# mozilla/mozjpeg

Hardware: AMD Instinct MI355X
Metric: Mpixels/s encode (4K RGB q75 trellis) at 1/2/4/8 GPUs; bit-exact vs cjpeg (higher is better)
Workload: dtype u8/int16 (+f32 trellis costs); 1 GPU; 3840x2160 synthetic RGB, q75 4:2:0 baseline, trellis+deringing+optimal Huffman (cjpeg -quality 75 -baseline); config_key=metric, frames_per_encode_call=96, distinct_frames=96, batches_in_flight=2, input=resident in HBM, output=complete JPEG files in HBM, parallelism=images sharded, 1 process per GPU, no collective

## Files before the change

### include/mozjpeg_hip.h

```cpp
#ifndef MOZJPEG_HIP_H
#define MOZJPEG_HIP_H

#include <stddef.h>
#include <stdint.h>

#ifdef __cplusplus
extern "C" {
#endif

#define MJH_MAX_COMPS 4
#define MJH_MAX_SCANS 64

#define MJH_OK            0
#define MJH_EINVAL       -1
#define MJH_EUNSUPPORTED -2
#define MJH_EHIP         -3
#define MJH_ENOMEM       -4
#define MJH_ETOOSMALL    -5

#define MJH_PROFILE_MAX_COMPRESSION 0x5D083AAD
#define MJH_PROFILE_FASTEST         0x2AEA5CB4

typedef struct {
  int comps_in_scan;
// ... 51 lines not shown

int mjh_std_huffman_table(int is_ac, int tblno, const uint8_t **bits, const uint8_t **vals, int *nvals);

int mjh_params_simple_progression(mjh_params *p);
int mjh_params_search_progression(mjh_params *p);

int mjh_encoder_create(const mjh_params *p, int max_batch, int device, mjh_encoder **out);
int mjh_device_count(void);
int mjh_device_numa_node(int device);
int mjh_bind_thread_to_device(int device);
int mjh_device_placement(int device, char *buf, size_t n);
void mjh_encoder_destroy(mjh_encoder *e);
const mjh_params *mjh_encoder_params(const mjh_encoder *e);

typedef struct mjh_pool mjh_pool;
int mjh_pool_create(const mjh_params *p, int max_batch_per_device, const int *devices, int ndevices, mjh_pool **out);
void mjh_pool_destroy(mjh_pool *pool);
int mjh_pool_device_count(const mjh_pool *pool);
int mjh_pool_encode_host(mjh_pool *pool, const void *pixels, size_t row_pitch, size_t image_stride, int n,
                         const uint8_t *const **jpegs, const size_t **sizes);
const char *mjh_pool_last_error(const mjh_pool *pool);

int mjh_encode_device(mjh_encoder *e, const void *d_pixels, size_t row_pitch, size_t image_stride,
                      int n, void *stream);
int mjh_set_inflight(mjh_encoder *e, int batches);
int mjh_encode_host(mjh_encoder *e, const void *pixels, size_t row_pitch, size_t image_stride, int n);
typedef struct { uint64_t offset, size; } mjh_result;
int mjh_collect(mjh_encoder *e, int age, const void **base, const mjh_result **results, int *count);
int mjh_wait_input(mjh_encoder *e);
int mjh_host_staging(mjh_encoder *e, void **buffer, size_t *bytes);
int mjh_stage_commit(mjh_encoder *e, size_t bytes);
int mjh_encode_gather(mjh_encoder *e, mjh_encoder *const *members, int n);
void *mjh_host_alloc(size_t bytes);
void mjh_host_free(void *p);
int mjh_host_register(void *p, size_t bytes);
int mjh_host_unregister(void *p);
int mjh_encode_planes_device(mjh_encoder *e, const void *const d_planes[MJH_MAX_COMPS], const size_t row_pitch[MJH_MAX_COMPS],
                             const size_t image_stride[MJH_MAX_COMPS], const int plane_width[MJH_MAX_COMPS],
                             const int plane_height[MJH_MAX_COMPS], int n, void *stream);
int mjh_encode_planes_host(mjh_encoder *e, const void *const planes[MJH_MAX_COMPS], const size_t row_pitch[MJH_MAX_COMPS],
                           const size_t image_stride[MJH_MAX_COMPS], const int plane_width[MJH_MAX_COMPS],
                           const int plane_height[MJH_MAX_COMPS], int n);
int mjh_encode_coefficients_device(mjh_encoder *e, const void *const d_coefs[MJH_MAX_COMPS], const size_t blocks_per_row[MJH_MAX_COMPS],
                                   const size_t image_stride[MJH_MAX_COMPS], int n, void *stream);
int mjh_encode_coefficients_host(mjh_encoder *e, const void *const coefs[MJH_MAX_COMPS], const size_t blocks_per_row[MJH_MAX_COMPS],
                                 const size_t image_stride[MJH_MAX_COMPS], int n);
int mjh_encoder_sync(mjh_encoder *e);

#define MJH_MAX_FILE_SCANS 4
#define MJH_CS_GRAYSCALE 1
#define MJH_CS_RGB       2
#define MJH_CS_YCbCr     3
typedef struct {
  int comps_in_scan;
  int component_index[MJH_MAX_COMPS];
  int dc_tbl_no[MJH_MAX_COMPS], ac_tbl_no[MJH_MAX_COMPS];
  unsigned restart_interval;
  size_t data_offset, data_size;
  unsigned restart_markers;
  int huff_defined;
  uint8_t huff_bits[8][17];
  uint8_t huff_vals[8][256];
} mjh_jpeg_scan;
typedef struct {
  int sof_type;
  int data_precision;
  int image_width, image_height;
  int num_components;
  int component_id[MJH_MAX_COMPS], h_samp_factor[MJH_MAX_COMPS], v_samp_factor[MJH_MAX_COMPS], quant_tbl_no[MJH_MAX_COMPS];
  int quant_defined;
  uint16_t quantval[4][64];
  int jpeg_color_space;
  int saw_JFIF_marker, JFIF_major_version, JFIF_minor_version, density_unit, X_density, Y_density;
  int saw_Adobe_marker, Adobe_transform;
  int num_scans;
  mjh_jpeg_scan scans[MJH_MAX_FILE_SCANS];
} mjh_jpeg_info;
int mjh_jpeg_probe(const void *jpeg, size_t size, mjh_jpeg_info *info);
int mjh_params_from_jpeg(const mjh_jpeg_info *info, int compress_profile, mjh_params *p);
int mjh_transcode_host(mjh_encoder *e, const void *const jpegs[], const size_t sizes[], int n);
int mjh_transcode_status(mjh_encoder *e, int i, const char **text);
int mjh_transcode_stats(mjh_encoder *e, int *subseq, int *rounds, int *host_syncs, float ms[4]);

int mjh_get_jpeg_size(mjh_encoder *e, int i, size_t *size);
int mjh_get_jpeg(mjh_encoder *e, int i, void *dst, size_t cap, size_t *size);
int mjh_get_output_device(mjh_encoder *e, void **d_base, size_t *stride, void **d_sizes);

int mjh_get_scan_table(mjh_encoder *e, int image, int scan, int tblno, uint8_t bits[17], uint8_t vals[256]);

enum {
  MJH_TAP_PLANE = 1,
  MJH_TAP_COEF_UQ = 2,
  MJH_TAP_COEF_Q = 3,
  MJH_TAP_COEF_Q0 = 4,
  MJH_TAP_HUFF_BITS = 5,
  MJH_TAP_HUFF_VALS = 6,
  MJH_TAP_PROG_SCAN_US = 7,
  MJH_TAP_LL_COUNTS = 8
};
int mjh_set_debug_taps(mjh_encoder *e, int on);
int mjh_read_tap(mjh_encoder *e, int what, int image, int component, void *dst, size_t cap, size_t *size);
int mjh_component_geometry(const mjh_encoder *e, int c, int *width_in_blocks, int *height_in_blocks,
                           int *plane_width, int *plane_height);

int mjh_set_profiling(mjh_encoder *e, int level);
int mjh_set_profiling_focus(mjh_encoder *e, const char *name);
int mjh_get_kernel_times(mjh_encoder *e, const char *const **names, const float **ms, int *count);

int mjh_debug_guard_mode(void);
int mjh_debug_guard_check(void);
int mjh_debug_guard_selftest(long offset, int write);

const char *mjh_last_error(void);
const char *mjh_version(void);
size_t mjh_params_size(void);

#ifdef __cplusplus
}
#endif
#endif
```

### mozjpeg_amd/__init__.py

```python
import ctypes as C
import os

import numpy as np

_HERE = os.path.dirname(os.path.abspath(__file__))
LIB_PATH = os.environ.get("MOZJPEG_AMD_LIB") or os.path.join(_HERE, "libmozjpeg_hip.so")

MAX_COMPS, MAX_SCANS = 4, 64
PROFILE_MAX_COMPRESSION = 0x5D083AAD
PROFILE_FASTEST = 0x2AEA5CB4
COLOR_YCC, COLOR_NONE, COLOR_YCC_IN = 0, 1, 2
CS_GRAYSCALE, CS_RGB, CS_YCBCR = 1, 2, 3
OK, EINVAL, EUNSUPPORTED, EHIP, ENOMEM, ETOOSMALL = 0, -1, -2, -3, -4, -5
TAP_PLANE, TAP_COEF_UQ, TAP_COEF_Q, TAP_COEF_Q0, TAP_HUFF_BITS, TAP_HUFF_VALS, TAP_PROG_SCAN_US, TAP_LL_COUNTS = 1, 2, 3, 4, 5, 6, 7, 8


class MjhError(RuntimeError):
    def __init__(self, code, msg):
        super().__init__("mozjpeg_hip error %d: %s" % (code, msg))
        self.code = code


class Scan(C.Structure):
    _fields_ = [("comps_in_scan", C.c_int), ("component_index", C.c_int * MAX_COMPS),
# ... 31 lines not shown
class JpegInfo(C.Structure):
    _fields_ = [("sof_type", C.c_int), ("data_precision", C.c_int), ("image_width", C.c_int), ("image_height", C.c_int),
                ("num_components", C.c_int), ("component_id", C.c_int * MAX_COMPS), ("h_samp_factor", C.c_int * MAX_COMPS),
                ("v_samp_factor", C.c_int * MAX_COMPS), ("quant_tbl_no", C.c_int * MAX_COMPS), ("quant_defined", C.c_int),
                ("quantval", (C.c_uint16 * 64) * 4), ("jpeg_color_space", C.c_int), ("saw_JFIF_marker", C.c_int),
                ("JFIF_major_version", C.c_int), ("JFIF_minor_version", C.c_int), ("density_unit", C.c_int),
                ("X_density", C.c_int), ("Y_density", C.c_int), ("saw_Adobe_marker", C.c_int), ("Adobe_transform", C.c_int),
                ("num_scans", C.c_int), ("scans", JpegScan * 4)]


class Result(C.Structure):
    _fields_ = [("offset", C.c_uint64), ("size", C.c_uint64)]


_lib = None


def lib():
    global _lib
    if _lib is None:
        if not os.path.exists(LIB_PATH):
            raise MjhError(EHIP, "%s not built: run `python -m mozjpeg_amd.build` (needs hipcc)" % LIB_PATH)
        L = C.CDLL(LIB_PATH)
        L.mjh_last_error.restype = C.c_char_p
        L.mjh_version.restype = C.c_char_p
        L.mjh_params_size.restype = C.c_size_t
        if L.mjh_params_size() != C.sizeof(Params):
            raise MjhError(EINVAL, "%s (%s) has a %d-byte mjh_params, this binding a %d-byte one: rebuild"
                           % (LIB_PATH, L.mjh_version().decode(), L.mjh_params_size(), C.sizeof(Params)))
        L.mjh_device_placement.argtypes = [C.c_int, C.c_char_p, C.c_size_t]
        L.mjh_params_defaults.argtypes = [C.POINTER(Params)] + [C.c_int] * 7
        L.mjh_params_set_quality.argtypes = [C.POINTER(Params), C.c_int, C.c_int, C.c_int]
        L.mjh_params_simple_progression.argtypes = [C.POINTER(Params)]
        L.mjh_params_search_progression.argtypes = [C.POINTER(Params)]
        L.mjh_encoder_create.argtypes = [C.POINTER(Params), C.c_int, C.c_int, C.POINTER(C.c_void_p)]
        L.mjh_encoder_destroy.argtypes = [C.c_void_p]
        L.mjh_encoder_destroy.restype = None
        L.mjh_encode_device.argtypes = [C.c_void_p, C.c_void_p, C.c_size_t, C.c_size_t, C.c_int, C.c_void_p]
        L.mjh_encode_host.argtypes = [C.c_void_p, C.c_void_p, C.c_size_t, C.c_size_t, C.c_int]
        L.mjh_encode_planes_device.argtypes = [C.c_void_p] + [C.c_void_p] * 5 + [C.c_int, C.c_void_p]
        L.mjh_encode_planes_host.argtypes = [C.c_void_p] + [C.c_void_p] * 5 + [C.c_int]
        L.mjh_encode_coefficients_device.argtypes = [C.c_void_p] + [C.c_void_p] * 3 + [C.c_int, C.c_void_p]
        L.mjh_encode_coefficients_host.argtypes = [C.c_void_p] + [C.c_void_p] * 3 + [C.c_int]
        L.mjh_encoder_sync.argtypes = [C.c_void_p]
        L.mjh_set_inflight.argtypes = [C.c_void_p, C.c_int]
        L.mjh_encoder_params.argtypes = [C.c_void_p]
        L.mjh_encoder_params.restype = C.POINTER(Params)
        L.mjh_pool_create.argtypes = [C.POINTER(Params), C.c_int, C.POINTER(C.c_int), C.c_int, C.POINTER(C.c_void_p)]
        L.mjh_pool_destroy.argtypes = [C.c_void_p]
        L.mjh_pool_destroy.restype = None
        L.mjh_pool_device_count.argtypes = [C.c_void_p]
        L.mjh_pool_encode_host.argtypes = [C.c_void_p, C.c_void_p, C.c_size_t, C.c_size_t, C.c_int,
                                           C.POINTER(C.POINTER(C.c_void_p)), C.POINTER(C.POINTER(C.c_size_t))]
        L.mjh_pool_last_error.argtypes = [C.c_void_p]
        L.mjh_pool_last_error.restype = C.c_char_p
        L.mjh_collect.argtypes = [C.c_void_p, C.c_int, C.POINTER(C.c_void_p), C.POINTER(C.POINTER(Result)), C.POINTER(C.c_int)]
        L.mjh_wait_input.argtypes = [C.c_void_p]
        L.mjh_host_staging.argtypes = [C.c_void_p, C.POINTER(C.c_void_p), C.POINTER(C.c_size_t)]
        L.mjh_stage_commit.argtypes = [C.c_void_p, C.c_size_t]
        L.mjh_encode_gather.argtypes = [C.c_void_p, C.POINTER(C.c_void_p), C.c_int]
        L.mjh_host_alloc.argtypes = [C.c_size_t]
        L.mjh_host_alloc.restype = C.c_void_p
        L.mjh_host_free.argtypes = [C.c_void_p]
        L.mjh_host_free.restype = None
        L.mjh_host_register.argtypes = [C.c_void_p, C.c_size_t]
        L.mjh_host_unregister.argtypes = [C.c_void_p]
        L.mjh_get_jpeg_size.argtypes = [C.c_void_p, C.c_int, C.POINTER(C.c_size_t)]
        L.mjh_get_jpeg.argtypes = [C.c_void_p, C.c_int, C.c_void_p, C.c_size_t, C.POINTER(C.c_size_t)]
        L.mjh_get_output_device.argtypes = [C.c_void_p, C.POINTER(C.c_void_p), C.POINTER(C.c_size_t),
                                            C.POINTER(C.c_void_p)]
        L.mjh_set_debug_taps.argtypes = [C.c_void_p, C.c_int]
        L.mjh_set_profiling.argtypes = [C.c_void_p, C.c_int]
        L.mjh_set_profiling_focus.argtypes = [C.c_void_p, C.c_char_p]
        L.mjh_read_tap.argtypes = [C.c_void_p, C.c_int, C.c_int, C.c_int, C.c_void_p, C.c_size_t,
                                   C.POINTER(C.c_size_t)]
        L.mjh_component_geometry.argtypes = [C.c_void_p, C.c_int] + [C.POINTER(C.c_int)] * 4
        L.mjh_get_kernel_times.argtypes = [C.c_void_p, C.POINTER(C.POINTER(C.c_char_p)),
                                           C.POINTER(C.POINTER(C.c_float)), C.POINTER(C.c_int)]
        L.mjh_jpeg_probe.argtypes = [C.c_char_p, C.c_size_t, C.POINTER(JpegInfo)]
        L.mjh_params_from_jpeg.argtypes = [C.POINTER(JpegInfo), C.c_int, C.POINTER(Params)]
        L.mjh_transcode_host.argtypes = [C.c_void_p, C.POINTER(C.c_char_p), C.POINTER(C.c_size_t), C.c_int]
        L.mjh_transcode_status.argtypes = [C.c_void_p, C.c_int, C.POINTER(C.c_char_p)]
        L.mjh_transcode_stats.argtypes = [C.c_void_p, C.POINTER(C.c_int), C.POINTER(C.c_int), C.POINTER(C.c_int), C.POINTER(C.c_float)]
        _lib = L
    return _lib


def _chk(rc):
    if rc != 0:
        raise MjhError(rc, lib().mjh_last_error().decode())


def make_params(width, height, *, quality=75, baseline=False, revert=False, optimize=False,
                notrellis=False, notrellis_dc=False, noovershoot=False, sample=(2, 2), gray=False,
                grayin=False, quant_table=-1, lambda1=None, lambda2=None, restart=None,
                progressive=False, fastcrush=False, precision=8, trellis_loops=1, smooth=0, rgb=False,
                dc_scan_opt=None, dc_ver_weight=None, use_scans_in_trellis=False, trellis_freq_split=0,
                trellis_eob_opt=False, trellis_q_opt=False, arithmetic=False, arith_cond=None, scans=None, gray_sample=None, yccin=False, dct=None,
                dc_tbl=None, ac_tbl=None, no_optimize=False, lossless=None):
    p = Params()
    L = lib()
    per_comp = isinstance(sample[0], (tuple, list))
    s0 = sample[0] if per_comp else sample
    _chk(L.mjh_params_defaults(C.byref(p), width, height, 1 if grayin else 3, 1 if gray else 0,
                               PROFILE_FASTEST if revert else PROFILE_MAX_COMPRESSION, s0[0], s0[1]))
    if per_comp and p.num_components == 3:
        for i in range(3):
            p.h_samp_factor[i], p.v_samp_factor[i] = sample[i]
    if gray_sample is not None and p.num_components == 1:
        p.h_samp_factor[0], p.v_samp_factor[0] = gray_sample
    _chk(L.mjh_params_set_quality(C.byref(p), quality, 1 if baseline else 0, quant_table))
    for i in range(p.num_components):
        if dc_tbl is not None:
            p.dc_tbl_no[i] = dc_tbl[i]
        if ac_tbl is not None:
            p.ac_tbl_no[i] = ac_tbl[i]
        for is_ac, t in ((0, p.dc_tbl_no[i]), (1, p.ac_tbl_no[i])):
            if t > 1 and (dc_tbl is not None or ac_tbl is not None):
                bits, vals, nv = C.POINTER(C.c_uint8)(), C.POINTER(C.c_uint8)(), C.c_int()
                _chk(L.mjh_std_huffman_table(is_ac, t & 1, C.byref(bits), C.byref(vals), C.byref(nv)))
                k = 2 * t + is_ac
                for j in range(17):
                    p.huff_bits[k][j] = bits[j]
                for j in range(nv.value):
                    p.huff_vals[k][j] = vals[j]
                p.huff_tables_given |= 1 << k
    if optimize:
        p.optimize_coding = 1
    if no_optimize:
        p.optimize_coding = 0
    if notrellis:
        p.trellis_quant = 0
    if notrellis_dc:
        p.trellis_quant_dc = 0
    if noovershoot:
        p.overshoot_deringing = 0
    if lambda1 is not None:
        p.lambda_log_scale1 = lambda1
    if lambda2 is not None:
        p.lambda_log_scale2 = lambda2
    p.data_precision = precision
    p.trellis_num_loops = trellis_loops
    p.smoothing_factor = smooth
    if dc_scan_opt is not None:
        p.dc_scan_opt_mode = dc_scan_opt
    if dc_ver_weight is not None:
        p.trellis_delta_dc_weight = dc_ver_weight
    p.use_scans_in_trellis = 1 if use_scans_in_trellis else 0
    p.trellis_freq_split = trellis_freq_split
    p.trellis_eob_opt = 1 if trellis_eob_opt else 0
    p.trellis_q_opt = 1 if trellis_q_opt else 0
    p.arith_code = 1 if arithmetic else 0
    if dct == "fast":
        p.dct_method = 1
    if arith_cond is not None:
        for t, (lo, up, kx) in enumerate(arith_cond):
            p.arith_dc_L[t], p.arith_dc_U[t], p.arith_ac_K[t] = lo, up, kx
    if yccin and not grayin:
        p.color_transform = COLOR_YCC_IN
    if rgb:
        p.color_transform = COLOR_NONE
        p.write_JFIF_header = 0
        for i, cid in enumerate(b"RGB"):
            p.component_id[i] = cid
            p.h_samp_factor[i] = p.v_samp_factor[i] = 1
            p.quant_tbl_no[i] = p.dc_tbl_no[i] = p.ac_tbl_no[i] = 0
# ... 212 lines not shown
        out = []
        for i in range(cnt.value):
            mv = (C.c_uint8 * res[i].size).from_address(base.value + res[i].offset)
            out.append(bytes(mv) if copy else memoryview(mv))
        return out

    def encode_device_ptr(self, ptr, row_pitch, image_stride, n, stream=None):
        _chk(lib().mjh_encode_device(self._h, ptr, row_pitch, image_stride, n, stream))

    def encode_tensor(self, t, stream=None):
        import torch
        p = self.params
        px = p.input_pixel_size or p.input_components
        es = 2 if p.data_precision > 8 else 1
        assert t.is_cuda and t.dim() == 4 and t.element_size() == es and t.stride(3) == 1 and t.stride(2) == t.shape[3], "layout"
        assert tuple(t.shape[1:]) == (p.image_height, p.image_width, px), "tensor %s does not match the encoder (%d x %d x %d)" % (
            tuple(t.shape), p.image_height, p.image_width, px)
        assert 1 <= t.shape[0] <= self.max_batch
        if stream is None:
            stream = torch.cuda.current_stream(t.device).cuda_stream or 1
        elif stream == "own":
            stream = None
        self.encode_device_ptr(t.data_ptr(), t.stride(1) * es, t.stride(0) * es, t.shape[0], stream)

    @staticmethod
    def _plane_args(ptrs, pitches, strides, widths, heights):
        k = len(ptrs)
        pad = lambda v, z: list(v) + [z] * (4 - k)
        return ((C.c_void_p * 4)(*pad(ptrs, None)), (C.c_size_t * 4)(*pad(pitches, 0)), (C.c_size_t * 4)(*pad(strides, 0)),
                (C.c_int * 4)(*pad(widths, 0)), (C.c_int * 4)(*pad(heights, 0)))

    def encode_planes_host(self, planes):
        dt = np.uint16 if self.params.data_precision == 12 else np.uint8
        arrs = [np.ascontiguousarray(a if a.ndim == 3 else a[None], dtype=dt) for a in planes]
        n = arrs[0].shape[0]
        args = self._plane_args([a.ctypes.data for a in arrs], [a.strides[1] for a in arrs], [a.strides[0] for a in arrs],
                                [a.shape[2] for a in arrs], [a.shape[1] for a in arrs])
        _chk(lib().mjh_encode_planes_host(self._h, *args, n))
        return [self.get_jpeg(i) for i in range(n)]

    def encode_planes_tensors(self, planes, stream=None):
        for t in planes:
            assert t.is_cuda and t.dim() == 3 and t.stride(2) == 1
        es = planes[0].element_size()
        n = planes[0].shape[0]
        args = self._plane_args([t.data_ptr() for t in planes], [t.stride(1) * es for t in planes],
                                [t.stride(0) * es for t in planes], [t.shape[2] for t in planes], [t.shape[1] for t in planes])
        _chk(lib().mjh_encode_planes_device(self._h, *args, n, stream))

    def encode_coefficients_host(self, coefs):
        arrs = [np.ascontiguousarray(a if a.ndim == 4 else a[None], dtype=np.int16) for a in coefs]
        n, k = arrs[0].shape[0], len(arrs)
        pad = lambda v, z: list(v) + [z] * (4 - k)
        _chk(lib().mjh_encode_coefficients_host(self._h, (C.c_void_p * 4)(*pad([a.ctypes.data for a in arrs], None)),
                                                (C.c_size_t * 4)(*pad([a.shape[2] for a in arrs], 0)),
                                                (C.c_size_t * 4)(*pad([a.strides[0] for a in arrs], 0)), n))
        return [self.get_jpeg(i) for i in range(n)]

    def encode_coefficients_tensors(self, coefs, stream=None):
        for t in coefs:
            assert t.is_cuda and t.is_contiguous() and t.dim() == 4 and t.element_size() == 2
        n, k = coefs[0].shape[0], len(coefs)
        pad = lambda v, z: list(v) + [z] * (4 - k)
        _chk(lib().mjh_encode_coefficients_device(self._h, (C.c_void_p * 4)(*pad([t.data_ptr() for t in coefs], None)),
                                                  (C.c_size_t * 4)(*pad([t.shape[2] for t in coefs], 0)),
                                                  (C.c_size_t * 4)(*pad([t.stride(0) * 2 for t in coefs], 0)), n, stream))

    def submit_transcode(self, files):
        files = [bytes(f) for f in files]
        n = len(files)
        _chk(lib().mjh_transcode_host(self._h, (C.c_char_p * n)(*files), (C.c_size_t * n)(*[len(f) for f in files]), n))
        return n

    def transcode_status(self, i):
        t = C.c_char_p()
        rc = lib().mjh_transcode_status(self._h, i, C.byref(t))
        return rc, (t.value or b"").decode()

    def transcode_stats(self):
        a, b, c, ms = C.c_int(), C.c_int(), C.c_int(), (C.c_float * 4)()
        _chk(lib().mjh_transcode_stats(self._h, C.byref(a), C.byref(b), C.byref(c), ms))
        return dict(subseq=a.value, rounds=b.value, host_syncs=c.value, ms=dict(zip(("sync", "prefix", "store", "dc"), [float(x) for x in ms])))

    def transcode_host(self, files, errors="raise"):
        n = len(files)
        try:
            self.submit_transcode(files)
            return [self.get_jpeg(i) for i in range(n)]
        except MjhError:
            if errors != "return":
                raise
            res = []
            for i in range(n):
                rc, text = self.transcode_status(i)
                res.append(MjhError(rc, text) if rc != OK else None)
            if all(r is None for r in res):
                raise
            return res

    def set_inflight(self, batches):
        _chk(lib().mjh_set_inflight(self._h, batches))

    def sync(self):
        _chk(lib().mjh_encoder_sync(self._h))

    def get_jpeg(self, i):
        n = C.c_size_t()
        _chk(lib().mjh_get_jpeg_size(self._h, i, C.byref(n)))
        buf = np.empty(n.value, np.uint8)
        _chk(lib().mjh_get_jpeg(self._h, i, buf.ctypes.data, n.value, C.byref(n)))
        return buf.tobytes()

    def jpeg_size(self, i):
        n = C.c_size_t()
        _chk(lib().mjh_get_jpeg_size(self._h, i, C.byref(n)))
        return n.value

    def set_debug_taps(self, on=True):
        _chk(lib().mjh_set_debug_taps(self._h, int(on)))

    def set_profiling(self, on=True, focus=None):
        if focus is not None:
            _chk(lib().mjh_set_profiling_focus(self._h, focus.encode()))
        _chk(lib().mjh_set_profiling(self._h, int(on)))

    def geometry(self, c):
        v = [C.c_int() for _ in range(4)]
        _chk(lib().mjh_component_geometry(self._h, c, *[C.byref(x) for x in v]))
        return tuple(x.value for x in v)

    def read_tap(self, what, image=0, comp=0):
        wib, hib, pw, ph = self.geometry(comp if what not in (TAP_HUFF_BITS, TAP_HUFF_VALS, TAP_PROG_SCAN_US) else 0)
        if what == TAP_PROG_SCAN_US:
            out = np.zeros((2, 72), np.uint32)
        elif what == TAP_PLANE:
            out = np.empty((ph, pw), np.uint8)
        elif what == TAP_HUFF_BITS:
            out = np.empty((4, 17), np.uint8)
        elif what == TAP_HUFF_VALS:
            out = np.empty((4, 256), np.uint8)
        else:
            out = np.empty((64, wib * hib), np.int16)
        n = C.c_size_t()
        _chk(lib().mjh_read_tap(self._h, what, image, comp, out.ctypes.data, out.nbytes, C.byref(n)))
        return out

    def kernel_times(self):
        names = C.POINTER(C.c_char_p)()
        ms = C.POINTER(C.c_float)()
        cnt = C.c_int()
        _chk(lib().mjh_get_kernel_times(self._h, C.byref(names), C.byref(ms), C.byref(cnt)))
        return [(names[i].decode(), float(ms[i])) for i in range(cnt.value)]
```

### mozjpeg_amd/csrc/mjh_device.h

```cpp
#ifndef MJH_DEVICE_H
#define MJH_DEVICE_H
#ifndef MJH_SIMT_HOST
#define MJH_DIVERGENT_SCOPE
#define MJH_WAVE_GROUPS(n) ((void)0)
#define MJH_WAVE_SYNC() ((void)0)
#define MJH_SCHED_BARRIER() __builtin_amdgcn_sched_barrier(0)
#endif
#include <hip/hip_runtime.h>
#include <stdint.h>
#include "mjh_internal.h"

__device__ __forceinline__ int bitlen(unsigned v) { return 32 - __clz((int)v); }

__device__ __forceinline__ int mul24(int a, int b) { return __mul24(a, b); }
__device__ __forceinline__ float squaref(int v) { const float f = (float)v; return f * f; }

__device__ __forceinline__ int udiv_exact(int n, int d, float rcp)
{
  int q = (int)((float)n * rcp);
  int r = n - mul24(q, d);
  if (r < 0) q--; else if (r >= d) q++;
  return q;
}

// ... 70 lines not shown
  return (unsigned)x;
}

__device__ __forceinline__ unsigned block_excl_scan_256_1b(unsigned v, unsigned *sh, int parity, unsigned *total)
{
  const int lane = threadIdx.x & 63, w = threadIdx.x >> 6;
  const unsigned inc = wave_incl_scan(v);
  if (lane == 63) sh[parity * 4 + w] = inc;
  __syncthreads();
  const unsigned a = sh[parity * 4], b = sh[parity * 4 + 1], c = sh[parity * 4 + 2], d = sh[parity * 4 + 3];
  *total = a + b + c + d;
  return (w == 0 ? 0u : (w == 1 ? a : (w == 2 ? a + b : a + b + c))) + inc - v;
}


struct BitWriter {
  unsigned *words;
  unsigned long long acc;
  int nacc;
  unsigned widx;
  __device__ __forceinline__ void init(unsigned *w, unsigned bitoff) { words = w; widx = bitoff >> 5; nacc = (int)(bitoff & 31); acc = 0; }
  __device__ __forceinline__ void put(unsigned code, int n)
  {
    acc = (acc << n) | (unsigned long long)(code & ((1u << n) - 1u));
    nacc += n;
    if (nacc >= 32) {
      const unsigned w = (unsigned)(acc >> (nacc - 32));
      atomicOr(&words[widx], __builtin_bswap32(w));
      widx++;
      nacc -= 32;
    }
  }
  __device__ __forceinline__ void put_sym(unsigned e, unsigned val, int nbits)
  {
    const int n = (int)(e >> 16) + nbits;
    acc = (acc << n) | (unsigned long long)(((e & 0xFFFFu) << nbits) | (val & ((1u << nbits) - 1u)));
    nacc += n;
    if (nacc >= 32) {
      const unsigned w = (unsigned)(acc >> (nacc - 32));
      atomicOr(&words[widx], __builtin_bswap32(w));
      widx++;
      nacc -= 32;
    }
  }
  __device__ __forceinline__ void flush()
  {
    if (nacc > 0) {
      const unsigned w = (unsigned)(acc << (32 - nacc));
      atomicOr(&words[widx], __builtin_bswap32(w));
    }
  }
};


#define STUFF_LDS_WORDS (4096 + 2)
__device__ __forceinline__ void stuff_store_round(uint8_t *__restrict__ o, unsigned dst0, unsigned total, unsigned my_dst, const unsigned (&w)[8],
                                                  int nvalid, unsigned keep, unsigned *lds)
{
  uint8_t *l8 = reinterpret_cast<uint8_t *>(lds);
  const unsigned shift = (unsigned)((uintptr_t)(o + dst0) & 3u);
  unsigned at = my_dst - dst0 + shift;
#pragma unroll
  for (int i = 0; i < 8; i++) {
#pragma unroll
    for (int b = 0; b < 4; b++) {
      const unsigned byte = (w[i] >> (8 * b)) & 0xFFu;
      if (4 * i + b < nvalid) {
        l8[at++] = (uint8_t)byte;
        if (byte == 0xFFu && !((keep >> (4 * i + b)) & 1u)) l8[at++] = 0;
      }
    }
  }
  __syncthreads();
  uint8_t *g = o + dst0 - shift;
  const unsigned end = shift + total, nw = (end + 3u) >> 2;
  for (unsigned k = threadIdx.x; k < nw; k += 256) {
    if (4 * k >= shift && 4 * k + 4 <= end) reinterpret_cast<unsigned *>(g)[k] = lds[k];
    else
      for (unsigned b = 4 * k; b < 4 * k + 4; b++) if (b >= shift && b < end) g[b] = l8[b];
  }
  __syncthreads();
}

template <bool LDSW>
struct BitSink {
  unsigned *words;
  unsigned long long acc;
  int nacc;
  unsigned widx;
  __device__ __forceinline__ void init(unsigned *w, unsigned bitoff) { words = w; widx = bitoff >> 5; nacc = (int)(bitoff & 31); acc = 0; }
  __device__ __forceinline__ void put(unsigned code, int n)
  {
    acc = (acc << n) | (unsigned long long)(code & ((1u << n) - 1u));
    nacc += n;
    if (nacc >= 32) {
      const unsigned w = (unsigned)(acc >> (nacc - 32));
      atomicOr(&words[widx], __builtin_bswap32(w));
      widx++;
      nacc -= 32;
    }
  }
  __device__ __forceinline__ void put_sym(unsigned e, unsigned val, int nbits)
  {
    const int n = (int)(e >> 16) + nbits;
    acc = (acc << n) | (unsigned long long)(((e & 0xFFFFu) << nbits) | (val & ((1u << nbits) - 1u)));
    nacc += n;
    if (nacc >= 32) {
      const unsigned w = (unsigned)(acc >> (nacc - 32));
      atomicOr(&words[widx], __builtin_bswap32(w));
      widx++;
      nacc -= 32;
    }
  }
  __device__ __forceinline__ void flush()
  {
    if (nacc > 0) atomicOr(&words[widx], __builtin_bswap32((unsigned)(acc << (32 - nacc))));
  }
  __device__ __forceinline__ unsigned bitpos() const { return widx * 32u + (unsigned)nacc; }
};

#endif
```

### mozjpeg_amd/csrc/mjh_encoder.cpp

```cpp
#include <hip/hip_runtime.h>

#include <math.h>
#include <stdarg.h>
#include <stdio.h>
#include <stdlib.h>
#include <string.h>

#include <atomic>
#include <condition_variable>
#include <functional>
#include <mutex>
#include <string>
#include <thread>
#include <memory>
#include <chrono>
#include <vector>

#include "../../include/mozjpeg_hip.h"
#include "mjh_internal.h"
#include "mjh_launch.h"
#include "mjh_lossless.h"
#include "mjh_decode.h"
#include "mjh_guard.h"
#include "mjh_numa.h"
// ... 211 lines not shown

enum { SLOTS_BASE = 16, SLOT_FINAL = 8, SLOT_PROG = 16 };


struct mjh_encoder {
  mjh_params p;
  MjhConst C;
  int device = 0;
  int max_batch = 0;
  int last_n = 0;
  hipStream_t stream = nullptr, copy_stream = nullptr, side_stream = nullptr;
  hipEvent_t copy_done = nullptr, ev_fork = nullptr, ev_join = nullptr, ev_side0 = nullptr, ev_side1 = nullptr;
  bool side_timed = false;
  uint8_t *d_pixb[2] = { nullptr, nullptr };
  uint8_t *h_stage[2] = { nullptr, nullptr };
  uint8_t *h_res[2] = { nullptr, nullptr };
  unsigned long long *h_tab[2] = { nullptr, nullptr };
  size_t res_cap = 0;
  hipEvent_t ev_h2d[2] = { nullptr, nullptr }, ev_pix_free[2] = { nullptr, nullptr }, ev_packed[2] = { nullptr, nullptr };
  hipStream_t d2h_stream = nullptr;
  unsigned host_calls = 0;
  size_t staged[2] = { 0, 0 };
  int res_buf = -1;
  int res_n[2] = { 0, 0 };
  bool res_waited[2] = { false, false };
  uint8_t *d_plin = nullptr, *h_plin = nullptr;
  uint8_t *d_cfin = nullptr, *h_cfin = nullptr;
  unsigned *d_prog_ffsums = nullptr;
  unsigned *d_prog_mpos = nullptr;
  int mpos_per_image = 0;
  size_t pix_image_bytes = 0;
  uint8_t *d_planes = nullptr;
  int16_t *d_uq = nullptr, *d_q = nullptr, *d_q0 = nullptr;
  MjhQuant *d_quant = nullptr, *d_quant_init = nullptr;
  MjhHuffTable *d_tabs = nullptr, *d_tabs_init = nullptr;
  float *d_lambda = nullptr;
  uint8_t *d_back = nullptr;
  void *d_eob_cost = nullptr; int *d_eob_has = nullptr; long long *d_qsums = nullptr;
  unsigned long long *d_nzmask = nullptr; bool use_compact = false, compact_last = false;
  size_t small_batch = 400000;
  uint8_t *d_nq8 = nullptr;
  int copy_prio = 0;
  int fastdiv_all = 0;
  int dc_mode = 0;
  int dc_late = 1;
  int dc_stats_side = 1;
  int dc_window_ok = 0;
  int trellis_chunks = 0;
  hipEvent_t ev_chunk[4] = { nullptr, nullptr, nullptr, nullptr };
  int trellis_v3 = 4;
  int dqt_off[4] = { -1, -1, -1, -1 };
  int dqt_tabs[4] = { 0, 0, 0, 0 }, dqt_ntab = 0;
  bool tbl_le1 = true;
  int nbands = 1, freq_split = 8;
  unsigned *d_seg_x = nullptr, *d_seg_E = nullptr, *d_seg_sums = nullptr, *d_seg_totals = nullptr, *d_mpos = nullptr;
  int nseg = 1;
  int comp_restart[4] = { 0, 0, 0, 0 };
  int16_t *d_dense = nullptr; unsigned dense_cap = 0;
  unsigned *d_worklist = nullptr, *d_worklist2 = nullptr;
  int trellis_variant = 0;
  bool trellis_adapt = true;
  int defer_scale = 1;
  unsigned *h_defer = nullptr;
  hipEvent_t ev_defer = nullptr; bool defer_pending = false; int defer_frames = 0;
  int spi = SLOTS_BASE;
  bool progressive = false;
  int nscans = 0;
  void *d_prog_scans = nullptr, *d_prog_ctl = nullptr;
  int *d_lists = nullptr;
  std::vector<int> h_lists;
  struct PList { int scan_off, nscan, slot_off, nslot, par_off, npar, nacf, seq_off, nseq; bool any_refine; };
  void *d_prog_chunks = nullptr;
  int chunks_per_scan = 0;
  MjhProgPE pe{};
  PList pl_trellis[2]{}, pl_phase[4]{}, pl_trellis_c[2][4]{};
  int nphases = 0;
  unsigned *d_pool = nullptr; size_t pool_words = 0;
  uint8_t *d_outpool = nullptr; size_t outpool_bytes = 0;
  uint8_t *d_frame_hdr = nullptr; int frame_hdr_len = 0, file_hdr_len = 0;
  uint16_t *d_len16 = nullptr;
  unsigned *d_off32 = nullptr, *d_sums = nullptr, *d_totals = nullptr, *d_ffsums = nullptr, *d_fftotals = nullptr;
  unsigned *d_stream = nullptr;
  size_t stream_words = 0;
  int chunks = 0, ff_chunks = 0;
  uint8_t *d_out = nullptr;
  size_t out_stride = 0;
  unsigned *d_sizes = nullptr;
  void *d_meta = nullptr;
  uint8_t *d_prefix = nullptr, *d_sos = nullptr;
  int prefix_len = 0, sos_len = 0;
  struct SeqScan { int ncomp; int comp[4]; int sos_off, sos_len; int dht_slots[8], dht_ids[8], ndht; int ri, nseg; };
  std::vector<SeqScan> seq_scans;
  int dht_slots[8] = { 0, 0, 0, 0, 0, 0, 0, 0 }, dht_ids[8] = { 0, 0, 0, 0, 0, 0, 0, 0 }, ndht = 0;
  bool debug_taps = false;
  int dc_chain_v = 1;
  int sof_hv0 = 0;
  bool fdct_div_zero = false;
  int profiling = 0;
  const char *prof_focus = "trellis_ac";
  std::string prof_focus_name;
  int prof_calls = 0;
  size_t prof_per_call = 0;
  std::vector<hipEvent_t> side_events;
  std::vector<std::string> prof_names;
  std::vector<const char *> prof_cnames;
  std::vector<float> prof_ms;
  std::vector<hipEvent_t> prof_events;
  std::vector<unsigned> h_sizes;
  bool sizes_valid = false;
  bool coef_input = false;
  hipStream_t last_stream = nullptr;
  mjh_params p_created;
  mjh_encoder *twin = nullptr;
  mjh_encoder *owner = nullptr;
  mjh_encoder *last = nullptr;
  int inflight = 2, inflight_mode = 1;
  unsigned dev_calls = 0;
  bool high_priority_streams = false;
  hipEvent_t ev_done = nullptr, ev_tier1 = nullptr;
  bool ev_done_set = false, ev_tier1_set = false;
  hipEvent_t ev_null_in = nullptr;
  uint8_t *d_back9 = nullptr; int *d_jfin = nullptr; int16_t *d_qspec = nullptr; int dc_spec = 1;
  bool arith = false;
  int arith_nscans = 0;
  void *d_arith_rates = nullptr;
  void *g_in[MJH_MAX_COMPS] = { nullptr, nullptr, nullptr, nullptr }; size_t g_in_bytes[MJH_MAX_COMPS] = { 0, 0, 0, 0 }; std::vector<void *> g_in_old;
  bool lossless = false;
  LlConst L{};
  unsigned *d_ll_hist = nullptr, *d_ll_len = nullptr, *d_ll_off = nullptr, *d_ll_segE = nullptr;
  int ll_sos_off[4] = { 0, 0, 0, 0 };
  int dec_subseq = 512;
  bool tc_preloaded = false;
  bool tc_batch[2] = { false, false };
  uint8_t *h_tc = nullptr, *d_tc = nullptr; size_t tc_cap = 0;
  uint8_t *h_tdesc = nullptr, *d_tdesc = nullptr; size_t tdesc_cap = 0;
  void *d_tsub = nullptr; size_t tsub_cap = 0;
  int16_t *d_tdiff = nullptr;
  unsigned *d_tstat = nullptr, *d_tchanged = nullptr, *h_tstat[2] = { nullptr, nullptr }, *h_tflag = nullptr;
  std::vector<int> tc_code; std::vector<std::string> tc_text;
  int tc_n = 0, tc_rounds = 0, tc_syncs = 0, tc_S = 0;
  bool tc_queued = false;
  hipEvent_t tc_ev[5] = { nullptr, nullptr, nullptr, nullptr, nullptr }; bool tc_timed = false;
};

static long div_round_up(long a, long b) { return (a + b - 1) / b; }

static int arith_qopt_passes(const mjh_params *p) { return (p->use_scans_in_trellis ? 2 : 1) * p->num_components * (p->trellis_num_loops > 1 ? p->trellis_num_loops : 1) + 1; }
static int arith_qopt_updates(const mjh_params *p) { return arith_qopt_passes(p) / ((p->use_scans_in_trellis ? 4 : 2) * p->num_components); }

static int dc_class(const mjh_params *p, int c)
{
  int seen[4], n = 0;
  for (int i = 0; i <= c; i++) {
    int k = 0;
    while (k < n && seen[k] != p->dc_tbl_no[i]) k++;
    if (k == n) seen[n++] = p->dc_tbl_no[i];
    if (i == c) return k;
  }
  return 0;
}

static bool trellis_without_optimize_is_optimize(const mjh_params *p)
{
  return p->num_components == 1 && p->num_scans == 0 && !p->use_scans_in_trellis && !(p->trellis_q_opt && p->trellis_num_loops > 1);
}

// ... 273 lines not shown
    o.push_back((uint8_t)((p->h_samp_factor[ci] << 4) + p->v_samp_factor[ci]));
    o.push_back((uint8_t)p->quant_tbl_no[ci]);
  }
}

static void build_sos(const mjh_params *p, int restart_interval, std::vector<uint8_t> &o)
{
  if (restart_interval) { o.push_back(0xFF); o.push_back(0xDD); put2(o, 4); put2(o, restart_interval); }
  o.push_back(0xFF); o.push_back(0xDA);
  put2(o, 2 * p->num_components + 2 + 1 + 3);
  o.push_back((uint8_t)p->num_components);
  for (int ci = 0; ci < p->num_components; ci++) {
    o.push_back((uint8_t)p->component_id[ci]);
    o.push_back((uint8_t)((p->dc_tbl_no[ci] << 4) + p->ac_tbl_no[ci]));
  }
  o.push_back(0); o.push_back(63); o.push_back(0);
}

static const uint8_t kStdDcLBits[17] = { 0, 0, 1, 5, 1, 1, 1, 1, 1, 1, 0, 0, 0, 0, 0, 0, 0 };
static const uint8_t kStdDcCBits[17] = { 0, 0, 3, 1, 1, 1, 1, 1, 1, 1, 1, 1, 0, 0, 0, 0, 0 };
static const uint8_t kStdDcVal[12] = { 0, 1, 2, 3, 4, 5, 6, 7, 8, 9, 10, 11 };
static const uint8_t kStdAcLBits[17] = { 0, 0, 2, 1, 3, 3, 2, 4, 3, 5, 5, 4, 4, 0, 0, 1, 0x7d };
static const uint8_t kStdAcLVal[162] = {
  0x01, 0x02, 0x03, 0x00, 0x04, 0x11, 0x05, 0x12, 0x21, 0x31, 0x41, 0x06, 0x13, 0x51, 0x61, 0x07,
  0x22, 0x71, 0x14, 0x32, 0x81, 0x91, 0xa1, 0x08, 0x23, 0x42, 0xb1, 0xc1, 0x15, 0x52, 0xd1, 0xf0,
  0x24, 0x33, 0x62, 0x72, 0x82, 0x09, 0x0a, 0x16, 0x17, 0x18, 0x19, 0x1a, 0x25, 0x26, 0x27, 0x28,
  0x29, 0x2a, 0x34, 0x35, 0x36, 0x37, 0x38, 0x39, 0x3a, 0x43, 0x44, 0x45, 0x46, 0x47, 0x48, 0x49,
  0x4a, 0x53, 0x54, 0x55, 0x56, 0x57, 0x58, 0x59, 0x5a, 0x63, 0x64, 0x65, 0x66, 0x67, 0x68, 0x69,
  0x6a, 0x73, 0x74, 0x75, 0x76, 0x77, 0x78, 0x79, 0x7a, 0x83, 0x84, 0x85, 0x86, 0x87, 0x88, 0x89,
  0x8a, 0x92, 0x93, 0x94, 0x95, 0x96, 0x97, 0x98, 0x99, 0x9a, 0xa2, 0xa3, 0xa4, 0xa5, 0xa6, 0xa7,
  0xa8, 0xa9, 0xaa, 0xb2, 0xb3, 0xb4, 0xb5, 0xb6, 0xb7, 0xb8, 0xb9, 0xba, 0xc2, 0xc3, 0xc4, 0xc5,
  0xc6, 0xc7, 0xc8, 0xc9, 0xca, 0xd2, 0xd3, 0xd4, 0xd5, 0xd6, 0xd7, 0xd8, 0xd9, 0xda, 0xe1, 0xe2,
  0xe3, 0xe4, 0xe5, 0xe6, 0xe7, 0xe8, 0xe9, 0xea, 0xf1, 0xf2, 0xf3, 0xf4, 0xf5, 0xf6, 0xf7, 0xf8,
  0xf9, 0xfa };
static const uint8_t kStdAcCBits[17] = { 0, 0, 2, 1, 2, 4, 4, 3, 4, 7, 5, 4, 4, 0, 1, 2, 0x77 };
static const uint8_t kStdAcCVal[162] = {
  0x00, 0x01, 0x02, 0x03, 0x11, 0x04, 0x05, 0x21, 0x31, 0x06, 0x12, 0x41, 0x51, 0x07, 0x61, 0x71,
  0x13, 0x22, 0x32, 0x81, 0x08, 0x14, 0x42, 0x91, 0xa1, 0xb1, 0xc1, 0x09, 0x23, 0x33, 0x52, 0xf0,
  0x15, 0x62, 0x72, 0xd1, 0x0a, 0x16, 0x24, 0x34, 0xe1, 0x25, 0xf1, 0x17, 0x18, 0x19, 0x1a, 0x26,
  0x27, 0x28, 0x29, 0x2a, 0x35, 0x36, 0x37, 0x38, 0x39, 0x3a, 0x43, 0x44, 0x45, 0x46, 0x47, 0x48,
  0x49, 0x4a, 0x53, 0x54, 0x55, 0x56, 0x57, 0x58, 0x59, 0x5a, 0x63, 0x64, 0x65, 0x66, 0x67, 0x68,
  0x69, 0x6a, 0x73, 0x74, 0x75, 0x76, 0x77, 0x78, 0x79, 0x7a, 0x82, 0x83, 0x84, 0x85, 0x86, 0x87,
  0x88, 0x89, 0x8a, 0x92, 0x93, 0x94, 0x95, 0x96, 0x97, 0x98, 0x99, 0x9a, 0xa2, 0xa3, 0xa4, 0xa5,
  0xa6, 0xa7, 0xa8, 0xa9, 0xaa, 0xb2, 0xb3, 0xb4, 0xb5, 0xb6, 0xb7, 0xb8, 0xb9, 0xba, 0xc2, 0xc3,
  0xc4, 0xc5, 0xc6, 0xc7, 0xc8, 0xc9, 0xca, 0xd2, 0xd3, 0xd4, 0xd5, 0xd6, 0xd7, 0xd8, 0xd9, 0xda,
  0xe2, 0xe3, 0xe4, 0xe5, 0xe6, 0xe7, 0xe8, 0xe9, 0xea, 0xf2, 0xf3, 0xf4, 0xf5, 0xf6, 0xf7, 0xf8,
  0xf9, 0xfa };

extern "C" int mjh_std_huffman_table(int is_ac, int tblno, const uint8_t **bits, const uint8_t **vals, int *nvals)
{
  if (!bits || !vals || !nvals || tblno < 0 || tblno > 1) return fail(MJH_EINVAL, "bad arguments");
  *bits = is_ac ? (tblno ? kStdAcCBits : kStdAcLBits) : (tblno ? kStdDcCBits : kStdDcLBits);
  *vals = is_ac ? (tblno ? kStdAcCVal : kStdAcLVal) : kStdDcVal;
  *nvals = is_ac ? 162 : 12;
  return MJH_OK;
}

static void fill_std_table(MjhHuffTable *T, const uint8_t *bits, const uint8_t *vals, int nvals)
{
  memset(T, 0, sizeof(*T));
  memcpy(T->bits, bits, 17);
  memcpy(T->huffval, vals, nvals);
  T->nsyms = nvals;
  int p = 0;
  unsigned code = 0;
  for (int l = 1; l <= 16; l++) {
    for (int i = 0; i < bits[l]; i++) {
      T->ehufsi[vals[p]] = (uint8_t)l;
      T->ehufco[vals[p]] = (uint16_t)code;
      code++; p++;
    }
    code <<= 1;
  }
}

static void free_all(mjh_encoder *e)
{
  if (!e) return;
  if (e->twin) { mjh_encoder *t = e->twin; e->twin = nullptr; free_all(t); }
  (void)hipSetDevice(e->device);
  for (hipEvent_t ev : { e->ev_done, e->ev_tier1 }) if (ev) (void)hipEventDestroy(ev);
  if (e->ev_null_in) (void)hipEventDestroy(e->ev_null_in);
  void *ptrs[] = { e->d_pixb[0], e->d_pixb[1], e->d_plin, e->d_cfin, e->d_prog_mpos, e->d_prog_ffsums, e->d_prog_chunks, e->pe.len16, e->pe.run16, e->pe.tail16, e->pe.be16, e->pe.off32, e->pe.sums, e->pe.totals, e->pe.T32, e->pe.tsums, e->pe.ttotals, e->pe.ne_bits, e->pe.ne2_bits, e->pe.e_bits, e->pe.info, e->pe.chist, e->pe.rmask, e->d_planes, e->d_uq, e->d_q, e->d_q0, e->d_quant, e->d_quant_init, e->d_tabs, e->d_tabs_init, e->d_lambda, e->d_back, e->d_eob_cost, e->d_eob_has, e->d_qsums, e->d_nzmask, e->d_nq8, e->d_dense, e->d_worklist, e->d_worklist2, e->d_prog_scans, e->d_prog_ctl, e->d_lists, e->d_pool, e->d_outpool, e->d_frame_hdr, e->d_seg_x, e->d_seg_E, e->d_seg_sums, e->d_seg_totals, e->d_mpos,
                   e->d_len16, e->d_off32, e->d_sums, e->d_totals, e->d_ffsums, e->d_fftotals, e->d_stream, e->d_out, e->d_sizes,
                   e->d_meta, e->d_prefix, e->d_sos, e->d_ll_hist, e->d_ll_len, e->d_ll_off, e->d_ll_segE, e->d_arith_rates, e->d_back9, e->d_jfin, e->d_qspec, e->g_in[0], e->g_in[1], e->g_in[2], e->g_in[3] };
  for (void *q : ptrs) if (q) (void)mjh_guard_free(q);
  for (void *q : e->g_in_old) (void)mjh_guard_free(q);
  if (e->ev_defer) (void)hipEventDestroy(e->ev_defer);
  if (e->h_defer) (void)hipHostFree(e->h_defer);
  for (int b = 0; b < 2; b++) {
    if (e->h_stage[b]) (void)hipHostFree(e->h_stage[b]);
    if (e->h_res[b]) (void)mjh_guard_host_free(e->h_res[b]);
    if (e->h_tab[b]) (void)mjh_guard_host_free(e->h_tab[b]);
    for (hipEvent_t ev : { e->ev_h2d[b], e->ev_pix_free[b], e->ev_packed[b] }) if (ev) (void)hipEventDestroy(ev);
  }
  if (e->d2h_stream) (void)hipStreamDestroy(e->d2h_stream);
  if (e->h_plin) (void)hipHostFree(e->h_plin);
  if (e->h_cfin) (void)hipHostFree(e->h_cfin);
  for (void *q : { (void *)e->d_tc, (void *)e->d_tdesc, e->d_tsub, (void *)e->d_tdiff, (void *)e->d_tstat, (void *)e->d_tchanged }) if (q) (void)mjh_guard_free(q);
  for (void *q : { (void *)e->h_tc, (void *)e->h_tdesc, (void *)e->h_tstat[0], (void *)e->h_tstat[1], (void *)e->h_tflag }) if (q) (void)hipHostFree(q);
  for (hipEvent_t ev : e->tc_ev) if (ev) (void)hipEventDestroy(ev);
  for (hipEvent_t ev : e->prof_events) (void)hipEventDestroy(ev);
  for (hipEvent_t ev : e->side_events) (void)hipEventDestroy(ev);
  if (e->copy_done) (void)hipEventDestroy(e->copy_done);
  for (hipEvent_t ev : { e->ev_fork, e->ev_join, e->ev_side0, e->ev_side1, e->ev_chunk[0], e->ev_chunk[1], e->ev_chunk[2], e->ev_chunk[3] }) if (ev) (void)hipEventDestroy(ev);
  if (e->side_stream) (void)hipStreamDestroy(e->side_stream);
  if (e->stream) (void)hipStreamDestroy(e->stream);
  if (e->copy_stream) (void)hipStreamDestroy(e->copy_stream);
  delete e;
}

extern "C" void mjh_encoder_destroy(mjh_encoder *e) { free_all(e); }

#define HIPCHK_E(x) do { hipError_t e_ = (x); if (e_ != hipSuccess) { int rc_ = fail(MJH_EHIP, "%s: %s (%s:%d)", #x, hipGetErrorString(e_), __FILE__, __LINE__); free_all(e); return rc_; } } while (0)

static MjhConst scan_view(const MjhConst &C, const mjh_params &p, const int *comps, int k)
{
  MjhConst V = C;
  V.ncomp = k;
  int mb = 0;
  for (int j = 0; j < k; j++) {
    V.c[j] = C.c[comps[j]];
    if (k == 1) {
      V.c[j].h = V.c[j].v = 1;
      V.c[j].wpad = V.c[j].wib; V.c[j].hpad = V.c[j].hib;
      V.mcus_per_row = V.c[j].wib; V.mcu_rows = V.c[j].hib;
    }
    V.c[j].mcu_blk0 = mb;
    mb += V.c[j].h * V.c[j].v;
  }
  V.blocks_per_mcu = mb;
  V.total_mcu_blocks = V.mcus_per_row * V.mcu_rows * mb;
  long ri = p.restart_interval;
  if (p.restart_in_rows > 0) { ri = (long)p.restart_in_rows * V.mcus_per_row; if (ri > 65535L) ri = 65535L; }
  V.restart_interval = (int)ri;
  return V;
}

static int mjh_streams_overlap(hipStream_t a, hipStream_t b)
{
  if (hipStreamSynchronize(a) != hipSuccess || hipStreamSynchronize(b) != hipSuccess) return -1;
  int votes = 0;
  for (int rep = 0; rep < 3; rep++) {
    const auto t0 = std::chrono::steady_clock::now();
    mjh_launch_spin(15000ull, a);
    mjh_launch_spin(15000ull, b);
    if (hipStreamSynchronize(a) != hipSuccess || hipStreamSynchronize(b) != hipSuccess) return -1;
    const double us = std::chrono::duration<double, std::micro>(std::chrono::steady_clock::now() - t0).count();
    votes += us < 240.0;
  }
  return votes >= 2;
}

static thread_local bool g_create_twin = false;
static thread_local hipStream_t g_twin_avoid[2] = { nullptr, nullptr };

static hipError_t make_streams(mjh_encoder *e)
{
#define STREAMCHK(x) do { const hipError_t r_ = (x); if (r_ != hipSuccess) return r_; } while (0)
  if (e->high_priority_streams) {
    std::vector<hipStream_t> made;
    for (int tries = 0; tries < 12 && !e->side_stream; tries++) {
      hipStream_t c = nullptr;
      STREAMCHK(hipStreamCreateWithFlags(&c, hipStreamNonBlocking));
      made.push_back(c);
      bool free_queue = true;
      for (hipStream_t other : { g_twin_avoid[0], g_twin_avoid[1], e->stream })
        if (other && mjh_streams_overlap(c, other) == 0) { free_queue = false; break; }
      if (!free_queue) continue;
      if (!e->stream) e->stream = c; else e->side_stream = c;
    }
    for (hipStream_t c : made) if (c != e->stream && c != e->side_stream) (void)hipStreamDestroy(c);
    if (!e->stream) STREAMCHK(hipStreamCreateWithFlags(&e->stream, hipStreamNonBlocking));
    if (!e->side_stream) STREAMCHK(hipStreamCreateWithFlags(&e->side_stream, hipStreamNonBlocking));
  } else {
    STREAMCHK(hipStreamCreateWithFlags(&e->stream, hipStreamNonBlocking));
    STREAMCHK(hipStreamCreateWithFlags(&e->side_stream, hipStreamNonBlocking));
  }
#undef STREAMCHK
  return hipSuccess;
}

static int create_lossless(const mjh_params *p, int max_batch, int device, mjh_encoder **out);

extern "C" int mjh_encoder_create(const mjh_params *p, int max_batch, int device, mjh_encoder **out)
{
  if (!p || !out || max_batch < 1) return fail(MJH_EINVAL, "bad arguments");
  *out = nullptr;
  if (p->num_scans > 0 && p->num_scans <= MJH_MAX_SCANS && p->scan_info[0].Ss != 0 && p->scan_info[0].Se == 0)
    return create_lossless(p, max_batch, device, out);
  mjh_params pn = *p;
  std::vector<mjh_scan> seq_script;
  if (p->num_scans > 0 && p->num_scans <= MJH_MAX_SCANS && !p->optimize_scans && p->scan_info[0].Ss == 0 && p->scan_info[0].Se == 63) {
    bool sent[MJH_MAX_COMPS] = { false, false, false, false };
    for (int si = 0; si < p->num_scans; si++) {
      const mjh_scan &sc = p->scan_info[si];
      if (sc.Ss != 0 || sc.Se != 63 || sc.Ah != 0 || sc.Al != 0) return fail(MJH_EINVAL, "scan %d: a sequential script holds whole-block scans only (Ss 0, Se 63, Ah 0, Al 0; JERR_BAD_PROG_SCRIPT)", si);
      if (sc.comps_in_scan < 1 || sc.comps_in_scan > p->num_components) return fail(MJH_EINVAL, "scan %d: component count", si);
      for (int ci = 0; ci < sc.comps_in_scan; ci++) {
        const int c = sc.component_index[ci];
        if (c < 0 || c >= p->num_components || (ci > 0 && c <= sc.component_index[ci - 1])) return fail(MJH_EINVAL, "scan %d: component order", si);
        if (sent[c]) return fail(MJH_EINVAL, "scan %d: component %d is coded twice (JERR_BAD_SCAN_SCRIPT)", si, c);
        sent[c] = true;
      }
      seq_script.push_back(sc);
    }
    for (int c = 0; c < p->num_components; c++) if (!sent[c]) return fail(MJH_EINVAL, "the script leaves component %d out (JERR_MISSING_DATA)", c);
    pn.num_scans = 0;
    if (seq_script.size() == 1) seq_script.clear();
    p = &pn;
  }
  if (p->arith_code && p->trellis_quant && p->trellis_q_opt && arith_qopt_updates(p) == 0) {
    if (p != &pn) { pn = *p; p = &pn; }
    pn.trellis_q_opt = 0;
  }
  int rc = check_supported(p);
  if (rc) return rc;
  if (!p->arith_code && p->compress_profile != MJH_PROFILE_FASTEST && p->num_scans == 0) {
    const int all[MJH_MAX_COMPS] = { 0, 1, 2, 3 };
    bool dseen[4] = { false, false, false, false }, aseen[4] = { false, false, false, false };
    bool bad = seq_script.empty() && dht_writer_would_corrupt(p, all, p->num_components, dseen, aseen);
    for (const mjh_scan &sc : seq_script) {
      if (p->optimize_coding || p->data_precision == 12) for (int t = 0; t < 4; t++) dseen[t] = aseen[t] = false;
      bad = bad || dht_writer_would_corrupt(p, sc.component_index, sc.comps_in_scan, dseen, aseen);
    }
    if (bad) return fail(MJH_EUNSUPPORTED, "dc_tbl_no / ac_tbl_no: a component reuses an earlier component's DC table with an AC table no earlier component had -- the reference's DHT writer (emit_multi_dht, jcmarker.c:293-401) writes a corrupt marker for this assignment");
  }
  int ndev = 0;
  if (hipGetDeviceCount(&ndev) != hipSuccess || ndev <= 0)
    return fail(MJH_EHIP, "no HIP device available: libmozjpeg_hip has no CPU fallback");
  if (device < 0 || device >= ndev) return fail(MJH_EINVAL, "device %d out of range (%d devices)", device, ndev);
  mjh_encoder *e = new mjh_encoder();
  e->p = *p;
  e->p_created = *p;
  e->high_priority_streams = g_create_twin;
  if (p->num_components == 1 && (p->h_samp_factor[0] != 1 || p->v_samp_factor[0] != 1)) {
    e->sof_hv0 = (p->h_samp_factor[0] << 4) + p->v_samp_factor[0];
    e->dc_chain_v = p->v_samp_factor[0];
    e->p.h_samp_factor[0] = e->p.v_samp_factor[0] = 1;
  }
  if (p->trellis_quant && !p->optimize_coding && !p->arith_code) e->p.optimize_coding = 1, e->p.huff_tables_given = 0;
  if (p->data_precision == 12 && !p->huff_tables_given) e->p.optimize_coding = 1;
  p = &e->p;
  e->device = device;
  e->max_batch = max_batch;
  build_const(p, &e->C);
  const MjhConst &C = e->C;
  e->progressive = p->num_scans > 0;
  e->nscans = p->num_scans;
  if (e->progressive) e->spi = SLOT_PROG + 2 * (p->num_scans + C.ncomp);
  e->nbands = p->trellis_quant && p->use_scans_in_trellis ? 2 : 1;
  e->freq_split = p->trellis_freq_split > 0 ? p->trellis_freq_split : 8;
  HIPCHK_E(hipSetDevice(device));
  HIPCHK_E(make_streams(e));
  HIPCHK_E(hipEventCreateWithFlags(&e->ev_done, hipEventDisableTiming));
  HIPCHK_E(hipEventCreateWithFlags(&e->ev_tier1, hipEventDisableTiming));
  if (const char *v = getenv("MJH_INFLIGHT")) { e->inflight = atoi(v); if (e->inflight < 1 || e->inflight > 2) e->inflight = 2; }
  if (const char *v = getenv("MJH_INFLIGHT_MODE")) { e->inflight_mode = atoi(v); if (e->inflight_mode < 0 || e->inflight_mode > 2) e->inflight_mode = 1; }
  {
    e->copy_prio = 0;
    HIPCHK_E(hipStreamCreateWithPriority(&e->copy_stream, hipStreamNonBlocking, e->copy_prio));
  }
  HIPCHK_E(hipEventCreateWithFlags(&e->copy_done, hipEventDisableTiming));
  HIPCHK_E(hipEventCreateWithFlags(&e->ev_fork, hipEventDisableTiming));
  HIPCHK_E(hipEventCreateWithFlags(&e->ev_join, hipEventDisableTiming));
  HIPCHK_E(hipEventCreate(&e->ev_side0));
  HIPCHK_E(hipEventCreate(&e->ev_side1));
  const size_t B = (size_t)max_batch;
  const size_t bps = C.precision == 12 ? 2 : 1;
  e->pix_image_bytes = (size_t)C.W * C.H * C.px_size * bps;
  HIPCHK_E(mjh_dmalloc((void **)&e->d_planes, B * C.planes_per_image * bps));
  HIPCHK_E(mjh_dmalloc((void **)&e->d_uq, B * C.coefs_per_image * 2));
  HIPCHK_E(mjh_dmalloc((void **)&e->d_q, B * C.coefs_per_image * 2));
  HIPCHK_E(mjh_dmalloc((void **)&e->d_quant, sizeof(MjhQuant) * (p->trellis_quant && p->trellis_q_opt ? B : 1)));
  HIPCHK_E(mjh_dmalloc((void **)&e->d_quant_init, sizeof(MjhQuant)));
  HIPCHK_E(mjh_dmalloc((void **)&e->d_tabs, B * e->spi * sizeof(MjhHuffTable)));
  HIPCHK_E(mjh_dmalloc((void **)&e->d_tabs_init, B * e->spi * sizeof(MjhHuffTable)));
  HIPCHK_E(mjh_dmalloc((void **)&e->d_lambda, B * C.total_real_blocks * sizeof(float)));
  HIPCHK_E(mjh_dmalloc((void **)&e->d_back, B * (size_t)C.total_real_blocks * 16));
  HIPCHK_E(mjh_dmalloc((void **)&e->d_worklist, 256 + B * (size_t)C.total_real_blocks * 12));
  HIPCHK_E(mjh_dmalloc((void **)&e->d_worklist2, 256 + B * (size_t)C.total_real_blocks * 12));
  if (p->trellis_quant && p->trellis_eob_opt) {
    HIPCHK_E(mjh_dmalloc(&e->d_eob_cost, B * (size_t)C.total_real_blocks * 8));
    HIPCHK_E(mjh_dmalloc((void **)&e->d_eob_has, B * (size_t)C.total_real_blocks * 4));
  }
  if (p->trellis_quant && p->trellis_q_opt) HIPCHK_E(mjh_dmalloc((void **)&e->d_qsums, B * 4 * 64 * 2 * sizeof(long long)));
  {
    const int nl = p->trellis_num_loops > 1 ? p->trellis_num_loops : 1;
    bool restart_scans = false;
    if (e->progressive && (p->restart_interval || p->restart_in_rows)) restart_scans = true;
    e->use_compact = !p->arith_code && p->trellis_quant && nl == 1 && e->nbands == 1 && !p->trellis_eob_opt && !p->trellis_q_opt &&
                     (e->progressive ? !restart_scans : true);
    if (e->use_compact) HIPCHK_E(mjh_dmalloc((void **)&e->d_nzmask, B * (size_t)C.total_real_blocks * sizeof(unsigned long long)));
    if (e->use_compact && p->trellis_quant) HIPCHK_E(mjh_dmalloc((void **)&e->d_nq8, B * (size_t)C.total_real_blocks));
  }
  if (p->trellis_quant) {
    e->dense_cap = (unsigned)(B * (size_t)C.total_real_blocks / 4 + 1024);
    if (const char *dv = getenv("MJH_DENSE_CAP")) e->dense_cap = (unsigned)atoi(dv) + 1u;
    HIPCHK_E(mjh_dmalloc((void **)&e->d_dense, (size_t)e->dense_cap * 128));
  }
  {
    double m = 0.0;
    for (int k = 1; k < 64; k++) m += p->quantval[p->quant_tbl_no[0]][k];
    m /= 63.0;
    e->trellis_variant = m >= 38.0 ? 0 : m >= 22.0 ? 2 : m >= 13.0 ? 3 : 4;
  }
  if (const char *v = getenv("MJH_TRELLIS_VARIANT")) { e->trellis_variant = atoi(v); e->trellis_adapt = false; }
  HIPCHK_E(hipHostMalloc((void **)&e->h_defer, 64, hipHostMallocDefault));
  if (const char *v = getenv("MJH_TRELLIS_V3")) e->trellis_v3 = atoi(v);
  if (const char *v = getenv("MJH_SMALL_BATCH")) e->small_batch = (size_t)atoll(v);
  if (const char *v = getenv("MJH_TRELLIS_CHUNKS")) { e->trellis_chunks = atoi(v); if (e->trellis_chunks < 0 || e->trellis_chunks > 4) e->trellis_chunks = 0; }
  for (int i = 0; i < 4; i++) HIPCHK_E(hipEventCreateWithFlags(&e->ev_chunk[i], hipEventDisableTiming));
  if (const char *v = getenv("MJH_DC_LATE")) { e->dc_late = atoi(v); if (e->dc_late < 0 || e->dc_late > 2) e->dc_late = 1; }
  e->dc_window_ok = 1;
  for (int i = 0; i < C.ncomp; i++) if (p->quantval[p->quant_tbl_no[i]][0] < 5) e->dc_window_ok = 0;
  if (const char *v = getenv("MJH_DC_SPEC")) e->dc_spec = atoi(v);
  if (const char *v = getenv("MJH_DECODE_SUBSEQ")) { e->dec_subseq = atoi(v); if (e->dec_subseq < 0 || (e->dec_subseq > 0 && e->dec_subseq < 16)) e->dec_subseq = 16; }
  HIPCHK_E(mjh_dmalloc((void **)&e->d_len16, B * (size_t)C.total_mcu_blocks * 2));
  HIPCHK_E(mjh_dmalloc((void **)&e->d_off32, B * (size_t)C.total_mcu_blocks * 4));
  e->chunks = (C.total_mcu_blocks + 2047) / 2048;
  size_t words = (size_t)C.total_mcu_blocks * (C.precision == 12 ? 61 : 53) + 64;
  if (C.restart_interval) words += (size_t)(C.mcus_per_row * C.mcu_rows) / C.restart_interval + 1;
  if (words > (size_t)1 << 27) words = (size_t)1 << 27;
  e->stream_words = (words + 63) & ~(size_t)63;
  e->ff_chunks = (int)((e->stream_words + 2047) / 2048);
  HIPCHK_E(mjh_dmalloc((void **)&e->d_sums, B * e->chunks * sizeof(unsigned)));
  HIPCHK_E(mjh_dmalloc((void **)&e->d_ffsums, B * e->ff_chunks * sizeof(unsigned)));
  HIPCHK_E(mjh_dmalloc((void **)&e->d_totals, B * sizeof(unsigned)));
  HIPCHK_E(mjh_dmalloc((void **)&e->d_fftotals, B * sizeof(unsigned)));
  HIPCHK_E(mjh_dmalloc((void **)&e->d_stream, B * e->stream_words * 4 + 4096));
  e->out_stride = ((size_t)2048 + 1024 * seq_script.size() + e->stream_words * 8 + 255) & ~(size_t)255;
  HIPCHK_E(mjh_dmalloc((void **)&e->d_out, B * e->out_stride));
  HIPCHK_E(mjh_dmalloc((void **)&e->d_sizes, B * sizeof(unsigned)));
  {
    const int nmcu = C.mcus_per_row * C.mcu_rows;
    e->nseg = C.restart_interval ? (nmcu + C.restart_interval - 1) / C.restart_interval : 1;
    int max_nseg = e->nseg;
    for (const mjh_scan &sc : seq_script) {
      const MjhConst V = scan_view(C, *p, sc.component_index, sc.comps_in_scan);
      const int nm = V.mcus_per_row * V.mcu_rows, ns1 = V.restart_interval ? (nm + V.restart_interval - 1) / V.restart_interval : 1;
      max_nseg = ns1 > max_nseg ? ns1 : max_nseg;
    }
    for (int i = 0; i < C.ncomp; i++) {
      long ri = p->restart_interval;
      if (p->restart_in_rows > 0) { ri = (long)p->restart_in_rows * C.c[i].wib; if (ri > 65535L) ri = 65535L; }
      e->comp_restart[i] = (int)ri;
    }
    const size_t ns = (size_t)max_nseg;
    HIPCHK_E(mjh_dmalloc((void **)&e->d_seg_x, B * ns * 4));
    HIPCHK_E(mjh_dmalloc((void **)&e->d_seg_E, B * ns * 4));
    HIPCHK_E(mjh_dmalloc((void **)&e->d_mpos, B * ns * 4));
    HIPCHK_E(mjh_dmalloc((void **)&e->d_seg_sums, B * ((ns + 2047) / 2048) * 4));
    HIPCHK_E(mjh_dmalloc((void **)&e->d_seg_totals, B * 4));
  }
  HIPCHK_E(mjh_dmalloc(&e->d_meta, B * sizeof(MjhImageMeta)));
  e->h_sizes.resize(B);

  MjhQuant hq;
  memset(&hq, 0, sizeof(hq));
  for (int t = 0; t < 4; t++)
    for (int k = 0; k < 64; k++) {
      const int q = p->quantval[t][kZZ[k]] ? p->quantval[t][kZZ[k]] : 1;
      hq.q[t][k] = (uint16_t)q;
      hq.dq8[t][k] = 8 * q;
      hq.rcp8q[t][k] = 1.0f / (float)(8 * q);
      hq.thr8[t][k] = (float)(8 * q - ((8 * q) >> 1));
      hq.lambda_tbl[t][k] = (float)(1.0 / (double)(q * q));
      {
        static const int aan[64] = { 16384, 22725, 21407, 19266, 16384, 12873, 8867, 4520, 22725, 31521, 29692, 26722, 22725, 17855, 12299, 6270,
                                     21407, 29692, 27969, 25172, 21407, 16819, 11585, 5906, 19266, 26722, 25172, 22654, 19266, 15137, 10426, 5315,
                                     16384, 22725, 21407, 19266, 16384, 12873, 8867, 4520, 12873, 17855, 16819, 15137, 12873, 10114, 6967, 3552,
                                     8867, 12299, 11585, 10426, 8867, 6967, 4799, 2446, 4520, 6270, 5906, 5315, 4520, 3552, 2446, 1247 };
        const int dc = p->dct_method == 1 ? (C.precision == 12 ? (int)(((long)q * aan[kZZ[k]] + 1024L) >> 11) : (int)((((long)q * aan[kZZ[k]] + 1024L) >> 11) & 0xFFFF))
                                          : C.precision == 12 ? 8 * q : (int)((8u * (unsigned)q) & 0xFFFFu);
        if (dc == 0)
          for (int i = 0; i < C.ncomp; i++) if (p->quant_tbl_no[i] == t) e->fdct_div_zero = true;
        hq.dqc8[t][k] = dc ? dc : 8;
        hq.rcpc8q[t][k] = 1.0f / (float)(dc ? dc : 8);
      }
      if (q <= 255) {
        const unsigned d = 8u * (unsigned)q;
        int b = 0;
        while ((d >> b) != 0) b++;
        const int kk = 22 + b < 32 ? 22 + b : 32;
        hq.mdiv[t][k] = (uint32_t)((1ull << kk) / d + 1ull);
        hq.sdiv[t][k] = 32 - kk;
      }
    }
  e->fastdiv_all = 1;
  for (int t = 0; t < 4; t++) {
    hq.fastdiv[t] = 1;
    for (int k = 0; k < 64; k++) if (hq.q[t][k] > 255) hq.fastdiv[t] = 0;
  }
  for (int i = 0; i < C.ncomp; i++) if (!hq.fastdiv[p->quant_tbl_no[i]]) e->fastdiv_all = 0;
  HIPCHK_E(hipMemcpy(e->d_quant, &hq, sizeof(hq), hipMemcpyHostToDevice));
  HIPCHK_E(hipMemcpy(e->d_quant_init, &hq, sizeof(hq), hipMemcpyHostToDevice));

  {
    std::vector<MjhHuffTable> ht(B * e->spi);
    memset(ht.data(), 0, ht.size() * sizeof(MjhHuffTable));
    if (!p->optimize_coding || p->num_scans > 0) {
      for (size_t b = 0; b < B; b++) {
        MjhHuffTable *T = &ht[b * e->spi + SLOT_FINAL];
        fill_std_table(&T[0], kStdDcLBits, kStdDcVal, 12);
        fill_std_table(&T[1], kStdAcLBits, kStdAcLVal, 162);
        fill_std_table(&T[2], kStdDcCBits, kStdDcVal, 12);
        fill_std_table(&T[3], kStdAcCBits, kStdAcCVal, 162);
        for (int k = 0; k < 8; k++)
          if (p->huff_tables_given >> k & 1) {
// ... 640 lines not shown
      const int v_rst[4] = { e->comp_restart[ci], 0, 0, 0 };
      for (int band = 0; band < nbands; band++) {
        int Ss, Se;
        band_limits(band, Ss, Se);
        if (Se < Ss) continue;
        const int rc = trellis_pass(CV, v_dc_seq, v_dc_prog, v_ac, v_rst, &e->pl_trellis_c[band][ci], Ss, Se, first_pass, loop == nloops - 1, 1);
        if (rc != MJH_OK) return rc;
        first_pass = false;
      }
      if ((u + 1) % C.ncomp == 0) { pr.mark("trellis_q_opt(tables)"); mjh_launch_qopt_update(e->d_qsums, e->d_quant, n, s); }
    }
  }
  if (e->progressive) {
    for (int ph = 0; ph < e->nphases; ph++) {
      const mjh_encoder::PList &pl = e->pl_phase[ph];
      static const char *const kStats[4] = { "prog_stats(A)", "prog_stats(A2)", "prog_stats(A3)", "prog_stats(B)" };
      static const char *const kTabs[4] = { "gen_tables(A)", "gen_tables(A2)", "gen_tables(A3)", "gen_tables(B)" };
      static const char *const kEnc[4] = { "prog_encode(A)", "prog_encode(A2)", "prog_encode(A3)", "prog_encode(B)" };
      const int pn = p.optimize_scans ? ph : 0;
      pr.mark(kStats[pn]);
      const bool both = pl.nseq > 0 && pl.npar > 0;
      hipStream_t ps = s;
      if (both) {
        HIPCHK(hipEventRecord(e->ev_fork, s));
        HIPCHK(hipStreamWaitEvent(e->side_stream, e->ev_fork, 0));
        ps = e->side_stream;
      }
      mjh_launch_prog_stats_par(C, e->d_prog_scans, e->d_lists + pl.par_off, pl.npar, e->d_prog_ctl, e->d_q, e->d_tabs, spi,
                                e->pe, pl.any_refine, nzm, n, ps, pl.nacf);
      if (both) HIPCHK(hipEventRecord(e->ev_join, e->side_stream));
      if (pl.nseq)
        mjh_launch_prog_stats(C, e->d_prog_scans, e->d_lists + pl.seq_off, pl.nseq, e->d_prog_ctl, e->d_q, e->d_tabs, spi, e->d_prog_mpos, e->mpos_per_image, n, s);
      if (both) HIPCHK(hipStreamWaitEvent(s, e->ev_join, 0));
      pr.mark(kTabs[pn]);
      mjh_launch_gen_tables_list(e->d_tabs, spi, e->d_lists + pl.slot_off, pl.nslot, n, s);
      pr.mark(kEnc[pn]);
      mjh_launch_prog_encode(C, e->d_prog_scans, e->d_lists + pl.scan_off, pl.nscan, e->d_lists + pl.seq_off, pl.nseq, e->d_lists + pl.par_off, pl.npar,
                             e->pe, e->d_prog_ctl, e->d_q, e->d_tabs, spi, e->d_pool, e->pool_words,
                             e->d_frame_hdr, e->frame_hdr_len, p.compress_profile != MJH_PROFILE_FASTEST, e->d_outpool, e->outpool_bytes,
                             e->d_prog_mpos, e->mpos_per_image, e->d_prog_ffsums, nzm, n, s, e->side_stream, e->ev_fork, e->ev_join, pl.nacf);
      if (p.optimize_scans) { pr.mark("prog_select"); mjh_launch_prog_select(e->d_prog_ctl, C.ncomp, ph, p.dc_scan_opt_mode, n, s); }
    }
    if (before_output) HIPCHK(hipStreamWaitEvent(s, before_output, 0));
    pr.mark("prog_concat");
    mjh_launch_prog_concat(e->d_prog_ctl, e->d_prefix, e->file_hdr_len, e->d_outpool, e->outpool_bytes, e->d_out, e->out_stride, e->d_sizes, n, s);
    if (ext_qopt) {
      pr.mark("trellis_q_opt(DQT)");
      mjh_launch_qopt_fix(e->d_quant, e->d_out, e->out_stride, e->d_sizes, e->file_hdr_len, e->prefix_len - (10 + 3 * C.ncomp), e->dqt_tabs, e->dqt_ntab,
                          p.compress_profile != MJH_PROFILE_FASTEST, !e->progressive && C.precision == 8 && e->tbl_le1, n, s);
    }
    pr.mark(nullptr);
    pr.finish();
    HIPCHK(hipGetLastError());
    return MJH_OK;
  }
  if (!e->seq_scans.empty() && !e->arith) {
    if (before_output) HIPCHK(hipStreamWaitEvent(s, before_output, 0));
    for (size_t si = 0; si < e->seq_scans.size(); si++) {
      const mjh_encoder::SeqScan &q = e->seq_scans[si];
      const MjhConst V = scan_view(C, p, q.comp, q.ncomp);
      int v_dc[4] = { 0, 0, 0, 0 }, v_ac[4] = { 0, 0, 0, 0 };
      for (int j = 0; j < q.ncomp; j++) { v_dc[j] = fin_dc[q.comp[j]]; v_ac[j] = fin_ac[q.comp[j]]; }
      if (p.optimize_coding) {
        HIPCHK(hipMemcpyAsync(e->d_tabs, e->d_tabs_init, (size_t)n * spi * sizeof(MjhHuffTable), hipMemcpyDeviceToDevice, s));
        pr.mark("stats_ac(final)");
        mjh_launch_stats_ac(V, e->d_q, nzm, e->d_tabs, spi, v_ac, 1, n, s);
        pr.mark("stats_dc(final)");
        mjh_launch_stats_dc(V, e->d_q, e->d_tabs, spi, v_dc, 1, zero4, n, s);
        pr.mark("gen_tables(final)");
        int slots[8], ns = 0;
        for (int j = 0; j < q.ncomp; j++) {
          bool have_d = false, have_a = false;
          for (int t = 0; t < ns; t++) { have_d = have_d || slots[t] == v_dc[j]; have_a = have_a || slots[t] == v_ac[j]; }
          if (!have_d) slots[ns++] = v_dc[j];
          if (!have_a) slots[ns++] = v_ac[j];
        }
        mjh_launch_gen_tables(e->d_tabs, spi, slots, ns, n, s);
      }
      pr.mark("header");
      mjh_launch_header(si == 0 ? e->d_prefix : nullptr, si == 0 ? e->prefix_len : 0, e->d_sos + q.sos_off, q.sos_len, e->d_tabs, spi, q.dht_slots, q.dht_ids, q.ndht,
                        p.compress_profile != MJH_PROFILE_FASTEST, e->d_out, e->out_stride, e->d_meta, n, s, si == 0 ? nullptr : e->d_sizes);
      pr.mark("huff_encode");
      mjh_launch_encode(V, e->d_q, nzm, e->d_tabs, spi, v_dc, v_ac, e->d_len16, e->d_off32, e->d_sums, e->chunks, e->d_totals,
                        e->d_stream, e->stream_words, e->d_meta, e->d_seg_x, e->d_seg_E, e->d_seg_sums, e->d_seg_totals, e->d_mpos, q.nseg, n, s);
      pr.mark("byte_stuff");
      mjh_launch_stuff(e->d_stream, e->stream_words, e->d_totals, e->d_ffsums, e->ff_chunks, e->d_fftotals, e->d_out, e->out_stride,
                       e->d_meta, e->d_sizes, e->d_mpos, q.nseg, n, s);
    }
  } else {
    if (p.optimize_coding) {
      pr.mark("stats_ac(final)");
      mjh_launch_stats_ac(C, e->d_q, nzm, e->d_tabs, spi, fin_ac, 1, n, s);
      if (!final_dc_counted) {
        pr.mark("stats_dc(final)");
        mjh_launch_stats_dc(C, e->d_q, e->d_tabs, spi, fin_dc, 1, zero4, n, s);
      }
      if (join_late) {
        pr.mark("join(trellis_dc)");
        HIPCHK(hipStreamWaitEvent(s, e->ev_join, 0));
      }
      pr.mark("gen_tables(final)");
      mjh_launch_gen_tables(e->d_tabs, spi, e->dht_slots, e->ndht, n, s);
    }
    if (before_output) HIPCHK(hipStreamWaitEvent(s, before_output, 0));
    pr.mark("header");
    mjh_launch_header(e->d_prefix, e->prefix_len, e->d_sos, e->sos_len, e->d_tabs, spi, e->dht_slots, e->dht_ids, e->ndht,
                      p.compress_profile != MJH_PROFILE_FASTEST, e->d_out, e->out_stride, e->d_meta, n, s);
    pr.mark("huff_encode");
    mjh_launch_encode(C, e->d_q, nzm, e->d_tabs, spi, fin_dc, fin_ac, e->d_len16, e->d_off32, e->d_sums, e->chunks, e->d_totals,
                      e->d_stream, e->stream_words, e->d_meta, e->d_seg_x, e->d_seg_E, e->d_seg_sums, e->d_seg_totals, e->d_mpos, e->nseg, n, s);
    if (if_mode == 2) { HIPCHK(hipEventRecord(e->ev_done, s)); e->ev_done_set = true; }
    pr.mark("byte_stuff");
    mjh_launch_stuff(e->d_stream, e->stream_words, e->d_totals, e->d_ffsums, e->ff_chunks, e->d_fftotals, e->d_out, e->out_stride,
                     e->d_meta, e->d_sizes, e->d_mpos, e->nseg, n, s);
  }
  if (ext_qopt) {
    pr.mark("trellis_q_opt(DQT)");
    mjh_launch_qopt_fix(e->d_quant, e->d_out, e->out_stride, e->d_sizes, e->file_hdr_len, e->prefix_len - (10 + 3 * C.ncomp), e->dqt_tabs, e->dqt_ntab,
                        p.compress_profile != MJH_PROFILE_FASTEST, !e->progressive && C.precision == 8 && e->tbl_le1, n, s);
  }
  pr.mark(nullptr);
  pr.finish();
  if (peer && !(if_mode == 2 && e->ev_done_set)) { HIPCHK(hipEventRecord(e->ev_done, s)); e->ev_done_set = true; }
  HIPCHK(hipGetLastError());
  return MJH_OK;
}

extern "C" const mjh_params *mjh_encoder_params(const mjh_encoder *e) { return e ? &e->p : nullptr; }

static mjh_encoder *cur(mjh_encoder *e) { return e && e->last ? e->last : e; }

extern "C" int mjh_set_inflight(mjh_encoder *e, int batches)
{
  if (!e || batches < 1 || batches > 2) return fail(MJH_EINVAL, "batches in flight: 1 or 2");
  e->inflight = batches;
  return MJH_OK;
}

static int make_twin(mjh_encoder *e)
{
  mjh_encoder *t = nullptr;
  g_create_twin = true;
  g_twin_avoid[0] = e->stream; g_twin_avoid[1] = e->side_stream;
  const int rc = mjh_encoder_create(&e->p_created, e->max_batch, e->device, &t);
  g_create_twin = false;
  if (rc) return rc;
  t->owner = e;
  t->inflight = 1;
  t->profiling = e->profiling; t->prof_focus_name = e->prof_focus_name; t->prof_focus = e->prof_focus;
  e->twin = t;
  return MJH_OK;
}

static int wait_pending_pack(mjh_encoder *e, hipStream_t s)
{
  if (e->res_buf >= 0 && !e->res_waited[e->res_buf]) HIPCHK(hipStreamWaitEvent(s, e->ev_packed[e->res_buf], 0));
  return MJH_OK;
}

static int guard_input(mjh_encoder *e, int slot, const void **p, size_t bytes)
{
  if (mjh_guard_mode() < 2 || !*p || !bytes) return MJH_OK;
  static const bool off = getenv("MJH_GUARD_INPUT") && atoi(getenv("MJH_GUARD_INPUT")) == 0;
  if (off) return MJH_OK;
  HIPCHK(hipDeviceSynchronize());
  if (e->g_in[slot] && e->g_in_bytes[slot] != bytes) { e->g_in_old.push_back(e->g_in[slot]); e->g_in[slot] = nullptr; }
  if (!e->g_in[slot]) HIPCHK(mjh_dmalloc(&e->g_in[slot], bytes));
  e->g_in_bytes[slot] = bytes;
  HIPCHK(hipMemcpy(e->g_in[slot], *p, bytes, hipMemcpyDeviceToDevice));
  HIPCHK(hipDeviceSynchronize());
  if (getenv("MJH_GUARD_VERIFY_COPY") && bytes <= ((size_t)1 << 28)) {
    std::vector<uint8_t> a(bytes), b(bytes);
    HIPCHK(hipMemcpy(a.data(), *p, bytes, hipMemcpyDeviceToHost));
    HIPCHK(hipMemcpy(b.data(), e->g_in[slot], bytes, hipMemcpyDeviceToHost));
    size_t bad = 0, first = 0;
    for (size_t i = 0; i < bytes; i++) if (a[i] != b[i]) { if (!bad) first = i; bad++; }
    fprintf(stderr, "guard_input: %zu bytes, %zu differ (first at %zu) src %p copy %p\n", bytes, bad, first, *p, e->g_in[slot]);
  }
  *p = e->g_in[slot];
  return MJH_OK;
}

extern "C" int mjh_encode_device(mjh_encoder *e, const void *d_pixels, size_t row_pitch, size_t image_stride, int n, void *stream)
{
  if (!e || !d_pixels || n < 1 || n > e->max_batch) return fail(MJH_EINVAL, "bad arguments (n=%d, max_batch=%d)", n, e ? e->max_batch : 0);
  {
    const size_t row_bytes = (size_t)e->C.W * e->C.px_size * (e->C.precision > 8 ? 2 : 1);
    if (row_pitch < row_bytes || (n > 1 && image_stride < row_pitch * (size_t)(e->C.H - 1) + row_bytes))
      return fail(MJH_EINVAL, "row_pitch %zu / image_stride %zu too small for %dx%d images of %zu-byte rows", row_pitch, image_stride, e->C.W, e->C.H, row_bytes);
  }
  HIPCHK(hipSetDevice(e->device));
  {
    const size_t row_bytes = (size_t)e->C.W * e->C.px_size * (e->C.precision > 8 ? 2 : 1);
    const int rg = guard_input(e, 0, &d_pixels, (size_t)(n - 1) * image_stride + (size_t)(e->C.H - 1) * row_pitch + row_bytes);
    if (rg) return rg;
  }
  hipStream_t s = stream ? (hipStream_t)stream : e->stream;
  if (stream == (void *)1) {
    if (!e->ev_null_in) HIPCHK(hipEventCreateWithFlags(&e->ev_null_in, hipEventDisableTiming));
    HIPCHK(hipEventRecord(e->ev_null_in, nullptr));
    s = e->stream;
    HIPCHK(hipStreamWaitEvent(s, e->ev_null_in, 0));
  }
  { const int rcw = wait_pending_pack(e, s); if (rcw) return rcw; }
  mjh_encoder *t = e;
  if (e->inflight > 1 && !stream && !e->debug_taps && mjh_guard_mode() == 0 && !e->owner) {
    if (!e->twin && make_twin(e) != MJH_OK) e->inflight = 1;
    if (e->twin && (e->dev_calls++ & 1u)) t = e->twin;
    if (t != e) s = t->stream;
  }
  const int rc = run_pipeline(t, d_pixels, row_pitch, image_stride, n, s);
  e->last = t == e ? nullptr : t;
  return rc;
}

namespace {
class CopyPool {
 public:
  static CopyPool &get() { static CopyPool *p = new CopyPool; return *p; }
  int threads() const { return nthreads_; }
  void run(int njobs, const std::function<void(int)> &fn)
  {
    if (njobs <= 0) return;
    if (nthreads_ <= 1 || njobs == 1) { for (int i = 0; i < njobs; i++) fn(i); return; }
    std::unique_lock<std::mutex> big(submit_);
// ... 679 lines not shown
  B.status = e->d_tstat;
  B.diff = e->d_tdiff;
  B.nsub_padded = (int)nsubp; B.nseg = (int)segs.size(); B.nscan = (int)scans.size(); B.n = n;
  B.S = S > 0 ? S : 1;
  const bool timed = e->profiling != 0;
  HIPCHK(hipMemsetAsync(e->d_q, 0, (size_t)n * C.coefs_per_image * 2, s));
  HIPCHK(hipMemsetAsync(e->d_tdiff, 0, (size_t)n * (size_t)C.total_mcu_blocks * 2, s));
  HIPCHK(hipMemsetAsync(e->d_tstat, 0, (size_t)n * 4, s));
  HIPCHK(hipMemsetAsync(e->d_meta, 0, (size_t)n * sizeof(MjhImageMeta), s));
  if (timed) HIPCHK(hipEventRecord(e->tc_ev[0], s));
  mjh_launch_dec_sync(C, B, 0, 1, s);
  for (int done = 0, group = 3; done < max_nsub - 1;) {
    const int g = group < max_nsub - 1 - done ? group : max_nsub - 1 - done;
    HIPCHK(hipMemsetAsync(e->d_tchanged, 0, 64 * 4, s));
    for (int q = 0; q < g; q++) mjh_launch_dec_sync(C, B, q, 0, s);
    done += g;
    e->tc_rounds += g;
    if (done >= max_nsub - 1) break;
    HIPCHK(hipMemcpyAsync(e->h_tflag, e->d_tchanged + (g - 1), 4, hipMemcpyDeviceToHost, s));
    HIPCHK(hipStreamSynchronize(s));
    e->tc_syncs++;
    if (!*(volatile unsigned *)e->h_tflag) break;
    group = group * 2 < 64 ? group * 2 : 64;
  }
  if (timed) HIPCHK(hipEventRecord(e->tc_ev[1], s));
  mjh_launch_dec_prefix(B, s);
  if (timed) HIPCHK(hipEventRecord(e->tc_ev[2], s));
  mjh_launch_dec_store(C, B, e->d_q, s);
  if (timed) HIPCHK(hipEventRecord(e->tc_ev[3], s));
  mjh_launch_dec_dc(C, B, e->d_q, s);
  mjh_launch_dec_scrub(C, B, e->d_q, e->d_meta, s);
  if (timed) { HIPCHK(hipEventRecord(e->tc_ev[4], s)); e->tc_timed = true; }
  HIPCHK(hipGetLastError());
  const int b = (int)(e->host_calls & 1u);
  e->host_calls++;
  MjhCoefSrc cs;
  memset(&cs, 0, sizeof(cs));
  e->tc_preloaded = true;
  rc = run_pipeline(e, nullptr, 0, 0, n, s, nullptr, &cs, nullptr, e->host_calls > 1 ? e->ev_packed[b ^ 1] : nullptr);
  e->tc_preloaded = false;
  if (rc) return rc;
  mjh_launch_dec_finish(e->d_tdesc + o_jfif, e->p.write_JFIF_header ? 1 : 0, e->d_out, e->out_stride, e->d_meta, e->d_tstat, n, s);
  HIPCHK(hipMemcpyAsync(e->h_tstat[b], e->d_tstat, (size_t)n * 4, hipMemcpyDeviceToHost, s));
  rc = queue_pack(e, b, n);
  if (rc) return rc;
  e->tc_batch[b] = true;
  e->tc_queued = true;
  return MJH_OK;
}

extern "C" int mjh_transcode_status(mjh_encoder *e, int i, const char **text)
{
  if (!e || i < 0 || i >= e->tc_n) return fail(MJH_EINVAL, "bad file index");
  if (text) *text = "";
  if (e->tc_code[(size_t)i] == MJH_OK && e->tc_queued && e->res_buf >= 0 && e->tc_batch[e->res_buf] && i < e->res_n[e->res_buf]) {
    HIPCHK(hipSetDevice(e->device));
    HIPCHK(hipEventSynchronize(e->ev_packed[e->res_buf]));
    const unsigned st = e->h_tstat[e->res_buf][i];
    if (st) {
      e->tc_code[(size_t)i] = MJH_EINVAL;
      e->tc_text[(size_t)i] = (st & MJH_DEC_CORRUPT) ? "Corrupt JPEG data: the entropy-coded data does not decode to the scan's blocks (premature end, extraneous bytes or a bad Huffman code; the reference warns: JWRN_HIT_MARKER / JWRN_EXTRANEOUS_DATA / JWRN_HUFF_BAD_CODE)"
                                                         : "a DCT coefficient out of range (JERR_BAD_DCT_COEF, jchuff.c:489,596,624)";
    }
  }
  if (text) *text = e->tc_text[(size_t)i].c_str();
  if (e->tc_code[(size_t)i] != MJH_OK) return fail(e->tc_code[(size_t)i], "file %d: %s", i, e->tc_text[(size_t)i].c_str());
  return MJH_OK;
}

extern "C" int mjh_transcode_stats(mjh_encoder *e, int *subseq, int *rounds, int *host_syncs, float ms[4])
{
  if (!e) return fail(MJH_EINVAL, "null encoder");
  if (subseq) *subseq = e->tc_S;
  if (rounds) *rounds = e->tc_rounds;
  if (host_syncs) *host_syncs = e->tc_syncs;
  if (ms) {
    for (int k = 0; k < 4; k++) ms[k] = 0.f;
    if (e->tc_timed) {
      HIPCHK(hipSetDevice(e->device));
      HIPCHK(hipEventSynchronize(e->tc_ev[4]));
      for (int k = 0; k < 4; k++) HIPCHK(hipEventElapsedTime(&ms[k], e->tc_ev[k], e->tc_ev[k + 1]));
    }
  }
  return MJH_OK;
}

extern "C" int mjh_encoder_sync(mjh_encoder *e)
{
  if (!e) return fail(MJH_EINVAL, "null encoder");
  HIPCHK(hipSetDevice(e->device));
  HIPCHK(hipStreamSynchronize(e->last_stream ? e->last_stream : e->stream));
  if (e->twin) HIPCHK(hipStreamSynchronize(e->twin->last_stream ? e->twin->last_stream : e->twin->stream));
  return guard_verify();
}

static int fetch_sizes(mjh_encoder *e)
{
  if (e->sizes_valid) return MJH_OK;
  if (e->res_buf >= 0) {
    int rc = wait_results(e, e->res_buf);
    if (rc) return rc;
    for (int i = 0; i < e->last_n; i++) e->h_sizes[i] = (unsigned)e->h_tab[e->res_buf][3 + 2 * i];
    e->sizes_valid = true;
    return MJH_OK;
  }
  HIPCHK(hipSetDevice(e->device));
  HIPCHK(hipDeviceSynchronize());
  { const int rg = guard_verify(); if (rg) return rg; }
  HIPCHK(hipMemcpy(e->h_sizes.data(), e->d_sizes, (size_t)e->last_n * sizeof(unsigned), hipMemcpyDeviceToHost));
  if (e->progressive || e->arith) {
    std::vector<MjhProgCtl> ctl(e->last_n);
    HIPCHK(hipMemcpy(ctl.data(), e->d_prog_ctl, (size_t)e->last_n * sizeof(MjhProgCtl), hipMemcpyDeviceToHost));
    for (int i = 0; i < e->last_n; i++)
      if (ctl[i].error) return fail(ctl[i].error == 1 ? MJH_ETOOSMALL : MJH_EHIP, "progressive encode of image %d failed (%s)", i,
                                    ctl[i].error == 1 ? "scan buffers exceed the bit-stream pool" : "internal: scan size prediction mismatch");
  }
  else {
    std::vector<MjhImageMeta> mt(e->last_n);
    HIPCHK(hipMemcpy(mt.data(), e->d_meta, (size_t)e->last_n * sizeof(MjhImageMeta), hipMemcpyDeviceToHost));
    for (int i = 0; i < e->last_n; i++)
      if (mt[i].total_bits == 0xFFFFFFFFu) return fail(MJH_ETOOSMALL, "entropy-coded data of image %d exceeds the 32-bit (2^32 bits = 512 MB) offset range of one scan", i);

  }
  if (e->coef_input) {
    std::vector<MjhImageMeta> mt(e->last_n);
    HIPCHK(hipMemcpy(mt.data(), e->d_meta, (size_t)e->last_n * sizeof(MjhImageMeta), hipMemcpyDeviceToHost));
    for (int i = 0; i < e->last_n; i++)
      if (mt[i].bad_coef) return fail(MJH_EINVAL, "image %d holds a DCT coefficient out of range (JERR_BAD_DCT_COEF, jchuff.c:489,596,624)", i);
  }
  e->sizes_valid = true;
  return MJH_OK;
}

extern "C" int mjh_get_jpeg_size(mjh_encoder *e, int i, size_t *size)
{
  e = cur(e);
  if (!e || !size || i < 0 || i >= e->last_n) return fail(MJH_EINVAL, "bad image index");
  int rc = fetch_sizes(e);
  if (rc) return rc;
  *size = e->h_sizes[i];
  return MJH_OK;
}

extern "C" int mjh_get_jpeg(mjh_encoder *e, int i, void *dst, size_t cap, size_t *size)
{
  e = cur(e);
  if (!e || !dst || i < 0 || i >= e->last_n) return fail(MJH_EINVAL, "bad image index");
  int rc = fetch_sizes(e);
  if (rc) return rc;
  const size_t n = e->h_sizes[i];
  if (size) *size = n;
  if (n > cap) return fail(MJH_ETOOSMALL, "output buffer too small: need %zu bytes", n);
  if (e->res_buf >= 0 && e->h_tab[e->res_buf][2 + 2 * i] != ~0ull) {
    memcpy(dst, e->h_res[e->res_buf] + e->h_tab[e->res_buf][2 + 2 * i], n);
    return MJH_OK;
  }
  HIPCHK(hipSetDevice(e->device));
  HIPCHK(hipMemcpy(dst, e->d_out + (size_t)i * e->out_stride, n, hipMemcpyDeviceToHost));
  return MJH_OK;
}

extern "C" int mjh_get_output_device(mjh_encoder *e, void **d_base, size_t *stride, void **d_sizes)
{
  e = cur(e);
  if (!e) return fail(MJH_EINVAL, "null encoder");
  if (d_base) *d_base = e->d_out;
// ... 406 lines not shown
```

### mozjpeg_amd/csrc/mjh_kernels.hip

```cpp
#include <hip/hip_runtime.h>
#include <stdio.h>
#include <stdlib.h>
#include <stdint.h>
#include <type_traits>
#include <stdlib.h>
#include "mjh_internal.h"
#include "mjh_device.h"

#define WAVE 64

struct ZZTab { int v[64]; };
static constexpr ZZTab make_zz() {
  ZZTab t{};
  const int z[64] = {
    0,  1,  8, 16,  9,  2,  3, 10, 17, 24, 32, 25, 18, 11,  4,  5,
    12, 19, 26, 33, 40, 48, 41, 34, 27, 20, 13,  6,  7, 14, 21, 28,
    35, 42, 49, 56, 57, 50, 43, 36, 29, 22, 15, 23, 30, 37, 44, 51,
    58, 59, 52, 45, 38, 31, 39, 46, 53, 60, 61, 54, 47, 55, 62, 63 };
  for (int i = 0; i < 64; i++) t.v[i] = z[i];
  return t;
}
static constexpr ZZTab kZZ = make_zz();

#define FIXC(x) ((int)((x) * 65536.0 + 0.5))
// ... 1627 lines not shown
  for (int i = 0; i < 8; i++) if (base + i < n_per_image) s += p[base + i];
  const unsigned tot = block_reduce_256(s, sh);
  if (threadIdx.x == 0) sums[(size_t)img * chunks_per_image + chunk] = tot;
}

__global__ void __launch_bounds__(256)
k_scan_sums(unsigned *__restrict__ sums, int chunks_per_image, unsigned *__restrict__ totals, const unsigned *__restrict__ stream_bits)
{
  __shared__ unsigned sh[4];
  const int img = blockIdx.x;
  unsigned *p = sums + (size_t)img * chunks_per_image;
  unsigned carry = 0;
  unsigned long long wide = 0;
  int nchunks = chunks_per_image;
  if (stream_bits) {
    const unsigned nwords = ((((stream_bits[img] + 7) >> 3) + 3) >> 2);
    nchunks = min(chunks_per_image, (int)((nwords + SCAN_CHUNK - 1) / SCAN_CHUNK));
  }
  for (int base = 0; base < nchunks; base += 256) {
    const int i = base + threadIdx.x;
    const unsigned v = i < nchunks ? p[i] : 0u;
    unsigned tot;
    const unsigned ex = block_excl_scan_256(v, sh, &tot);
    if (i < nchunks) p[i] = carry + ex;
    carry += tot;
    wide += tot;
  }
  if (threadIdx.x == 0) totals[img] = wide >= 0xFFF00000ull ? 0xFFFFFFFFu : carry;
}

template <class T>
__global__ void __launch_bounds__(256)
k_offsets(const T *__restrict__ len16, int n_per_image, const unsigned *__restrict__ sums,
          int chunks_per_image, unsigned *__restrict__ off32)
{
  __shared__ unsigned sh[4];
  const int img = blockIdx.y, chunk = blockIdx.x;
  const T *p = len16 + (size_t)img * n_per_image;
  unsigned *o = off32 + (size_t)img * n_per_image;
  const int base = chunk * SCAN_CHUNK + threadIdx.x * 8;
  unsigned v[8], s = 0;
#pragma unroll
  for (int i = 0; i < 8; i++) { v[i] = base + i < n_per_image ? p[base + i] : 0u; s += v[i]; }
  unsigned ex = block_excl_scan_256(s, sh, nullptr) + sums[(size_t)img * chunks_per_image + chunk];
#pragma unroll
  for (int i = 0; i < 8; i++) { if (base + i < n_per_image) o[base + i] = ex; ex += v[i]; }
}

__global__ void __launch_bounds__(256)
k_seg_extra(MjhConst C, const unsigned *__restrict__ off32, const unsigned *__restrict__ totals,
            unsigned *__restrict__ seg_x, int nseg)
{
  const int img = blockIdx.y;
  const int sidx = blockIdx.x * 256 + threadIdx.x;
  if (sidx >= nseg) return;
  const unsigned *o = off32 + (size_t)img * C.total_mcu_blocks;
  const long long per = (long long)C.restart_interval * C.blocks_per_mcu;
  const long long bs = sidx * per, be = bs + per;
  const unsigned start = o[bs];
  const unsigned end = be < C.total_mcu_blocks ? o[be] : totals[img];
  const unsigned L = end - start;
  seg_x[(size_t)img * nseg + sidx] = sidx < nseg - 1 ? ((8u - (L & 7u)) & 7u) + 16u : 0u;
}

struct MarkerCursor {
  const unsigned *mpos; int n, idx;
  __device__ __forceinline__ MarkerCursor(const unsigned *m, int nmark) : mpos(m), n(nmark), idx(-1) {}
  __device__ __forceinline__ bool at(unsigned bytepos)
  {
    if (idx < 0) {
      int lo = 0, hi = n;
      while (lo < hi) { const int mid = (lo + hi) >> 1; if (mpos[mid] < bytepos) lo = mid + 1; else hi = mid; }
      idx = lo;
    }
    while (idx < n && mpos[idx] < bytepos) idx++;
    return idx < n && mpos[idx] == bytepos;
  }
};

#define ENCW_WIN 4096

template <bool COMPACT, class W>
__device__ __forceinline__ void enc_write_block(const MjhConst &C, const MjhComp &cc, W &bw, const unsigned *s_ac, const unsigned *s_dc,
                                                const int16_t *__restrict__ q, const unsigned long long *__restrict__ nzmask_img, int r, int c)
{
  const int dc = q[dc_source_block(cc, r, c)];
  int pr, pc, pred = 0;
  if (mcu_prev_block(C, cc, r, c, pr, pc)) pred = q[dc_source_block(cc, pr, pc)];
  {
    const int df = dc - pred;
    const int a = df < 0 ? -df : df;
    const int nb = bitlen((unsigned)a);
    const unsigned e = s_dc[nb];
    bw.put(e & 0xFFFF, (int)(e >> 16));
    if (nb) bw.put((unsigned)(df < 0 ? df - 1 : df), nb);
  }
  const bool real = r < cc.hib && c < cc.wib;
  const int b = real ? r * cc.wib + c : 0;
  if (COMPACT) {
    const unsigned long long m = nzmask_img[cc.blk_off + b];
    int prev = 0;
    for_each_nonzero(q + b, (size_t)cc.kstride, m, real, [&](int pos, int v) {
      int run = pos - prev - 1;
      prev = pos;
      while (run > 15) { const unsigned e = s_ac[0xF0]; bw.put(e & 0xFFFF, (int)(e >> 16)); run -= 16; }
      const int a = v < 0 ? -v : v;
      const int nbv = bitlen((unsigned)a);
      const unsigned e = s_ac[(run << 4) + nbv];
      bw.put_sym(e, (unsigned)(v < 0 ? v - 1 : v), nbv);
    });
    if (!real || prev < 63) { const unsigned e = s_ac[0]; bw.put(e & 0xFFFF, (int)(e >> 16)); }
  } else {
    int x[64];
#pragma unroll
    for (int k = 1; k < 64; k++) x[k] = q[(size_t)k * cc.kstride + b];
    if (real) {
      int run = 0;
#pragma unroll
      for (int k = 1; k < 64; k++) {
        const int v = x[k];
        if (v == 0) run++;
        else {
          while (run > 15) { const unsigned e = s_ac[0xF0]; bw.put(e & 0xFFFF, (int)(e >> 16)); run -= 16; }
          const int a = v < 0 ? -v : v;
          const int nb = bitlen((unsigned)a);
          const unsigned e = s_ac[(run << 4) + nb];
          bw.put_sym(e, (unsigned)(v < 0 ? v - 1 : v), nb);
          run = 0;
        }
      }
      if (run > 0) { const unsigned e = s_ac[0]; bw.put(e & 0xFFFF, (int)(e >> 16)); }
    } else {
      const unsigned e = s_ac[0];
      bw.put(e & 0xFFFF, (int)(e >> 16));
    }
  }
}

template <bool COMPACT>
__global__ void __launch_bounds__(256)
k_enc_write_mcu(MjhConst C, const int16_t *__restrict__ coef_q, const unsigned long long *__restrict__ nzmask, const MjhHuffTable *__restrict__ tabs,
                int slots_per_image, int4 dc_slot_of_comp, int4 ac_slot_of_comp,
                const unsigned *__restrict__ off32, unsigned *__restrict__ stream, size_t stream_words_per_image,
                const unsigned *__restrict__ totals, const unsigned *__restrict__ seg_E, const unsigned *__restrict__ seg_totals,
                unsigned *__restrict__ mpos, int nseg)
{
  __shared__ unsigned s_ac[MJH_MAXC][256];
  __shared__ unsigned s_dc[MJH_MAXC][32];
  __shared__ unsigned s_win[ENCW_WIN];
  const int img = blockIdx.y, tid = threadIdx.x;
  const int N = C.total_mcu_blocks, base = blockIdx.x * 256;
  if (totals[img] == 0xFFFFFFFFu) return;
  for (int ci = 0; ci < C.ncomp; ci++) {
    const int dslot = ci == 0 ? dc_slot_of_comp.x : ci == 1 ? dc_slot_of_comp.y : ci == 2 ? dc_slot_of_comp.z : dc_slot_of_comp.w;
    const int aslot = ci == 0 ? ac_slot_of_comp.x : ci == 1 ? ac_slot_of_comp.y : ci == 2 ? ac_slot_of_comp.z : ac_slot_of_comp.w;
    const MjhHuffTable *TD = tabs + (size_t)img * slots_per_image + dslot;
    const MjhHuffTable *TA = tabs + (size_t)img * slots_per_image + aslot;
    s_ac[ci][tid] = ((unsigned)TA->ehufsi[tid] << 16) | TA->ehufco[tid];
    if (tid < 32) s_dc[ci][tid] = tid < 16 ? ((unsigned)TD->ehufsi[tid] << 16) | TD->ehufco[tid] : 0u;
  }
  auto final_off = [&](int p) -> unsigned {
    if (p >= N) return totals[img] + (nseg > 1 ? seg_totals[img] : 0u);
    const int mcu = p / C.blocks_per_mcu;
    return off32[(size_t)img * N + p] + (nseg > 1 ? seg_E[(size_t)img * nseg + mcu / C.restart_interval] : 0u);
  };
  const unsigned start = final_off(base), end = final_off(min(base + 256, N));
  const unsigned w0 = start >> 5, nw = ((end + 31u) >> 5) - w0;
  const bool window = nw <= (unsigned)ENCW_WIN;
  if (window) for (unsigned i = tid; i < nw; i += 256) s_win[i] = 0u;
  __syncthreads();
  unsigned *g = stream + (size_t)img * stream_words_per_image;
  const int p = base + tid;
  if (p < N) {
    const int mcu = p / C.blocks_per_mcu, bi = p - mcu * C.blocks_per_mcu;
    int comp = 0;
    for (int ci = 1; ci < C.ncomp; ci++) if (bi >= C.c[ci].mcu_blk0) comp = ci;
    const MjhComp cc = C.c[comp];
    const int local = bi - cc.mcu_blk0, yi = local / cc.h, xi = local - yi * cc.h;
    const int mrow = mcu / C.mcus_per_row, mcol = mcu - mrow * C.mcus_per_row;
    const int r = mrow * cc.v + yi, c = mcol * cc.h + xi;
    const int16_t *q = coef_q + (size_t)img * C.coefs_per_image + cc.coef_off;
    const unsigned long long *nzi = COMPACT ? nzmask + (size_t)img * C.total_real_blocks : nullptr;
    const unsigned fo = final_off(p);
    const int segi = C.restart_interval ? mcu / C.restart_interval : 0;
    const bool seg_end = C.restart_interval && segi < nseg - 1 && (mcu + 1) % C.restart_interval == 0 && bi == C.blocks_per_mcu - 1;
    auto emit = [&](auto &bw, unsigned wbase) {
      enc_write_block<COMPACT>(C, cc, bw, s_ac[comp], s_dc[comp], q, nzi, r, c);
      if (seg_end) {
        const unsigned bitpos = bw.bitpos() + wbase;
        const int pad = (int)((8u - (bitpos & 7u)) & 7u);
        if (pad) bw.put((1u << pad) - 1u, pad);
        mpos[(size_t)img * nseg + segi] = (bitpos + (unsigned)pad) >> 3;
        bw.put(0xFFD0u + (unsigned)(segi & 7), 16);
      }
      bw.flush();
    };
    if (window) { BitSink<true> bw; bw.init(s_win, fo - (w0 << 5)); emit(bw, w0 << 5); }
    else { BitSink<false> bw; bw.init(g, fo); emit(bw, 0u); }
  }
  __syncthreads();
  if (window)
    for (unsigned i = tid; i < nw; i += 256) {
      const unsigned v = s_win[i];
      if (v == 0u) continue;
      if (i == 0u || i == nw - 1u) atomicOr(&g[w0 + i], v);
      else g[w0 + i] = v;
    }
}

__global__ void __launch_bounds__(256)
k_zero_stream(unsigned *__restrict__ stream, size_t stream_words_per_image, const unsigned *__restrict__ totals,
              const unsigned *__restrict__ seg_totals)
{
  const int img = blockIdx.y;
  if (totals[img] == 0xFFFFFFFFu) return;
  const unsigned bits = totals[img] + (seg_totals ? seg_totals[img] : 0u);
  const unsigned nvec = ((bits >> 5) + 8) >> 2;
  uint4 *p = reinterpret_cast<uint4 *>(stream + (size_t)img * stream_words_per_image);
  for (unsigned i = blockIdx.x * 256 + threadIdx.x; i <= nvec; i += gridDim.x * 256) p[i] = make_uint4(0, 0, 0, 0);
}


__global__ void __launch_bounds__(64)
k_header(const uint8_t *__restrict__ prefix, int prefix_len, const uint8_t *__restrict__ sos, int sos_len,
         const MjhHuffTable *__restrict__ tabs, int slots_per_image, MjhDhtPlan dht, int ndht,
         int multi_dht, uint8_t *__restrict__ out, size_t out_stride, MjhImageMeta *__restrict__ meta, const unsigned *__restrict__ append_sizes)
{
  const int img = blockIdx.x;
  const int lane = threadIdx.x;
  uint8_t *o = out + (size_t)img * out_stride;
  const int start = append_sizes ? (int)append_sizes[img] - 2 : 0;
  for (int i = lane; i < prefix_len; i += 64) o[start + i] = prefix[i];
  int pos = start + prefix_len;
  const int *slots = dht.slots, *ids = dht.ids;
  if (multi_dht) {
    int length = 2;
    for (int i = 0; i < ndht; i++) length += (int)tabs[(size_t)img * slots_per_image + slots[i]].nsyms + 17;
    if (lane == 0) { o[pos] = 0xFF; o[pos + 1] = 0xC4; o[pos + 2] = (uint8_t)(length >> 8); o[pos + 3] = (uint8_t)length; }
    pos += 4;
  }
  for (int i = 0; i < ndht; i++) {
    const MjhHuffTable *T = tabs + (size_t)img * slots_per_image + slots[i];
    const int n = (int)T->nsyms;
    if (!multi_dht) {
      const int length = n + 2 + 1 + 16;
      if (lane == 0) { o[pos] = 0xFF; o[pos + 1] = 0xC4; o[pos + 2] = (uint8_t)(length >> 8); o[pos + 3] = (uint8_t)length; }
      pos += 4;
    }
    if (lane == 0) o[pos] = (uint8_t)ids[i];
    if (lane < 16) o[pos + 1 + lane] = T->bits[lane + 1];
    for (int j = lane; j < n; j += 64) o[pos + 17 + j] = T->huffval[j];
    pos += 17 + n;
  }
  for (int i = lane; i < sos_len; i += 64) o[pos + i] = sos[i];
  pos += sos_len;
  if (lane == 0) meta[img].hdr_len = (unsigned)pos;
}

__global__ void __launch_bounds__(64)
k_finish_bits(unsigned *__restrict__ totals, const unsigned *__restrict__ seg_totals, unsigned *__restrict__ stream,
              size_t stream_words_per_image, MjhImageMeta *__restrict__ meta, int nimg)
{
  const int img = blockIdx.x * 64 + threadIdx.x;
  if (img >= nimg) return;
  if (totals[img] == 0xFFFFFFFFu) {
    totals[img] = 0;
    meta[img].total_bits = 0xFFFFFFFFu;
    return;
  }
  const unsigned tb = totals[img] + (seg_totals ? seg_totals[img] : 0u);
  totals[img] = tb;
  meta[img].total_bits = tb;
  if (tb & 7) {
    const unsigned padbits = 8 - (tb & 7);
    const unsigned bitpos = tb & 31;
    const unsigned w = (((1u << padbits) - 1u) << (32 - bitpos - padbits));
    atomicOr(&stream[(size_t)img * stream_words_per_image + (tb >> 5)], __builtin_bswap32(w));
  }
}

__device__ __forceinline__ unsigned ff_count(unsigned w)
{
  unsigned c = 0;
  c += ((w & 0xFFu) == 0xFFu);
  c += ((w & 0xFF00u) == 0xFF00u);
  c += ((w & 0xFF0000u) == 0xFF0000u);
  c += ((w & 0xFF000000u) == 0xFF000000u);
  return c;
}

__global__ void __launch_bounds__(256)
k_ff_chunk_sums(const unsigned *__restrict__ stream, size_t stream_words_per_image, const unsigned *__restrict__ totals,
// ... 98 lines not shown
      }
      table[1] = err;
    }
  }
  if (!fits) return;
  const uint4 *src = reinterpret_cast<const uint4 *>(out + (size_t)img * out_stride);
  uint4 *d = reinterpret_cast<uint4 *>(dst + off);
  const unsigned nvec = (sz + 15u) >> 4;
  for (unsigned i = blockIdx.x * 256 + threadIdx.x; i < nvec; i += gridDim.x * 256) d[i] = src[i];
}

#include "mjh_launch.h"

static inline dim3 g3(unsigned x, unsigned y, unsigned z) { return dim3(x, y, z); }

void mjh_launch_pack_results(const void *out, size_t out_stride, const unsigned *sizes, const void *meta, const void *prog_ctl, int n,
                             void *dst, size_t cap, void *table, hipStream_t s)
{
  hipLaunchKernelGGL(k_pack_results, dim3(16, n), dim3(256), 0, s, (const uint8_t *)out, out_stride, sizes, (const MjhImageMeta *)meta,
                     (const MjhProgCtl *)prog_ctl, n, (uint8_t *)dst, cap, (unsigned long long *)table);
}

void mjh_launch_import_coefs(const MjhConst &C, const MjhCoefSrc &S, void *coef_q, void *meta, int n, hipStream_t s)
{
  (void)hipMemsetAsync(meta, 0, (size_t)n * sizeof(MjhImageMeta), s);
  int m = 0;
  for (int i = 0; i < C.ncomp; i++) m = C.c[i].nblk > m ? C.c[i].nblk : m;
  dim3 grid((m + 63) / 64, C.ncomp, n);
  hipLaunchKernelGGL(k_import_coefs, grid, dim3(64), 0, s, C, S, (int16_t *)coef_q, (MjhImageMeta *)meta);
}

void mjh_launch_import_planes(const MjhConst &C, const MjhPlaneSrc &S, void *planes, int n, hipStream_t s)
{
  int pw = 0, ph = 0;
  for (int i = 0; i < C.ncomp; i++) { pw = C.c[i].pw > pw ? C.c[i].pw : pw; ph = C.c[i].ph > ph ? C.c[i].ph : ph; }
  dim3 grid((pw / 4 + 255) / 256, ph, n * C.ncomp);
  if (C.precision == 12) hipLaunchKernelGGL((k_import_planes<uint16_t>), grid, dim3(256), 0, s, C, S, (uint16_t *)planes);
  else hipLaunchKernelGGL((k_import_planes<uint8_t>), grid, dim3(256), 0, s, C, S, (uint8_t *)planes);
}

void mjh_launch_color(const MjhConst &C, const void *pix, size_t row_pitch, size_t img_stride, void *planes, int n, hipStream_t s)
{
  const int H0 = C.maxh, V0 = C.maxv;
  if (C.smoothing) {
    int pw = 0, ph = 0;
    for (int i = 0; i < C.ncomp; i++) { pw = C.c[i].pw > pw ? C.c[i].pw : pw; ph = C.c[i].ph > ph ? C.c[i].ph : ph; }
    dim3 grid((pw + 255) / 256, ph, n * C.ncomp);
    if (C.precision == 12) hipLaunchKernelGGL((k_color_smooth<uint16_t>), grid, dim3(256), 0, s, C, (const uint8_t *)pix, row_pitch, img_stride, (uint16_t *)planes);
    else hipLaunchKernelGGL((k_color_smooth<uint8_t>), grid, dim3(256), 0, s, C, (const uint8_t *)pix, row_pitch, img_stride, (uint8_t *)planes);
    return;
  }
  bool plain = true;
  for (int i = 0; i < C.ncomp; i++) plain = plain && (i == 0 ? (C.c[i].h == H0 && C.c[i].v == V0) : (C.c[i].h == 1 && C.c[i].v == 1));
  plain = plain && (H0 == 1 || H0 == 2 || H0 == 4) && (V0 == 1 || V0 == 2 || V0 == 4);
  if (!plain) {
    int pw = 0, ph = 0;
    for (int i = 0; i < C.ncomp; i++) { pw = C.c[i].pw > pw ? C.c[i].pw : pw; ph = C.c[i].ph > ph ? C.c[i].ph : ph; }
    dim3 grid((pw + 255) / 256, ph, n * C.ncomp);
    if (C.precision == 12) hipLaunchKernelGGL((k_color_generic<uint16_t>), grid, dim3(256), 0, s, C, (const uint8_t *)pix, row_pitch, img_stride, (uint16_t *)planes);
    else hipLaunchKernelGGL((k_color_generic<uint8_t>), grid, dim3(256), 0, s, C, (const uint8_t *)pix, row_pitch, img_stride, (uint8_t *)planes);
    return;
  }
  if (!C.no_ycc && C.precision == 8 && C.in_comps == 3 && C.ncomp == 3 && C.px_size == 3 && H0 == 2 && V0 <= 2 && (row_pitch & 7) == 0 &&
      (img_stride & 7) == 0 && ((uintptr_t)pix & 7) == 0 && C.off_g == 1 && (C.off_r == 0 || C.off_r == 2)) {
    dim3 gridv(((C.groups_x + 3) / 4 + 255) / 256, C.groups_y, n);
    if (V0 == 2) hipLaunchKernelGGL((k_color_vec<2>), gridv, dim3(256), 0, s, C, (const uint8_t *)pix, row_pitch, img_stride, (uint8_t *)planes);
    else hipLaunchKernelGGL((k_color_vec<1>), gridv, dim3(256), 0, s, C, (const uint8_t *)pix, row_pitch, img_stride, (uint8_t *)planes);
    return;
  }
  dim3 grid((C.groups_x + 255) / 256, C.groups_y, n);
#define LC(h, v) do { if (C.precision == 12) hipLaunchKernelGGL((k_color<h, v, uint16_t>), grid, dim3(256), 0, s, C, (const uint8_t *)pix, row_pitch, img_stride, (uint16_t *)planes); \
                      else hipLaunchKernelGGL((k_color<h, v, uint8_t>), grid, dim3(256), 0, s, C, (const uint8_t *)pix, row_pitch, img_stride, (uint8_t *)planes); } while (0)
  if (H0 == 2 && V0 == 2) LC(2, 2);
  else if (H0 == 2 && V0 == 1) LC(2, 1);
  else if (H0 == 1 && V0 == 2) LC(1, 2);
  else if (H0 == 4 && V0 == 1) LC(4, 1);
  else if (H0 == 1 && V0 == 4) LC(1, 4);
  else if (H0 == 4 && V0 == 2) LC(4, 2);
  else if (H0 == 2 && V0 == 4) LC(2, 4);
  else LC(1, 1);
#undef LC
}

static int max_nblk(const MjhConst &C) { int m = 0; for (int i = 0; i < C.ncomp; i++) m = C.c[i].nblk > m ? C.c[i].nblk : m; return m; }
static int max_padblk(const MjhConst &C) { int m = 0; for (int i = 0; i < C.ncomp; i++) { int v = C.c[i].wpad * C.c[i].hpad; m = v > m ? v : m; } return m; }

void mjh_launch_dct(const MjhConst &C, const MjhQuant *Q, const void *planes, void *uq, void *q, float *lambda,
                    MjhHuffTable *stat_tabs, int spi, const int stat_slot[4], uint8_t *nq8, int n, hipStream_t s, int fastdiv, int ifast)
{
  const int nb = (stat_tabs && C.precision != 12) ? DCTQ_NB : 1;
  dim3 grid(((max_nblk(C) + 63) / 64 + nb - 1) / nb, C.ncomp, n);
  const int4 sl = stat_tabs ? make_int4(stat_slot[0], stat_slot[1], stat_slot[2], stat_slot[3]) : make_int4(0, 0, 0, 0);
  if (ifast && C.precision == 12) hipLaunchKernelGGL(k_dct_quant_ifast12, grid, dim3(64), 0, s, C, Q, (const uint16_t *)planes, (int16_t *)uq, (int16_t *)q, lambda, nq8);
  else if (ifast) hipLaunchKernelGGL(k_dct_quant_ifast, grid, dim3(64), 0, s, C, Q, (const uint8_t *)planes, (int16_t *)uq, (int16_t *)q, lambda, nq8);
  else if (C.precision == 12) hipLaunchKernelGGL((k_dct_quant<uint16_t, false>), grid, dim3(64), 0, s, C, Q, (const uint16_t *)planes, (int16_t *)uq, (int16_t *)q, lambda, stat_tabs, spi, sl, nq8);
  else if (stat_tabs && fastdiv) hipLaunchKernelGGL((k_dct_quant<uint8_t, true, true>), grid, dim3(64), 0, s, C, Q, (const uint8_t *)planes, (int16_t *)uq, (int16_t *)q, lambda, stat_tabs, spi, sl, nq8);
  else if (stat_tabs) hipLaunchKernelGGL((k_dct_quant<uint8_t, true>), grid, dim3(64), 0, s, C, Q, (const uint8_t *)planes, (int16_t *)uq, (int16_t *)q, lambda, stat_tabs, spi, sl, nq8);
  else if (fastdiv) hipLaunchKernelGGL((k_dct_quant<uint8_t, false, true>), grid, dim3(64), 0, s, C, Q, (const uint8_t *)planes, (int16_t *)uq, (int16_t *)q, lambda, stat_tabs, spi, sl, nq8);
  else hipLaunchKernelGGL((k_dct_quant<uint8_t, false>), grid, dim3(64), 0, s, C, Q, (const uint8_t *)planes, (int16_t *)uq, (int16_t *)q, lambda, stat_tabs, spi, sl, nq8);
}

void mjh_launch_stats_ac(const MjhConst &C, const void *q, const unsigned long long *nzmask, MjhHuffTable *tabs, int spi, const int slot[4], int count_dummies, int n, hipStream_t s)
{
  dim3 grid((max_nblk(C) + 255) / 256, C.ncomp, n), gridc((max_nblk(C) + 256 * STATS_AC_ITER - 1) / (256 * STATS_AC_ITER), C.ncomp, n);
  if (nzmask) hipLaunchKernelGGL(k_stats_ac_compact, gridc, dim3(256), 0, s, C, (const int16_t *)q, nzmask, tabs, spi, make_int4(slot[0], slot[1], slot[2], slot[3]), count_dummies);
  else hipLaunchKernelGGL(k_stats_ac, grid, dim3(256), 0, s, C, (const int16_t *)q, tabs, spi, make_int4(slot[0], slot[1], slot[2], slot[3]), count_dummies);
}

void mjh_launch_stats_dc(const MjhConst &C, const void *q, MjhHuffTable *tabs, int spi, const int slot[4], int mcu_order, const int comp_restart[4], int n, hipStream_t s)
{
  const int4 sl = make_int4(slot[0], slot[1], slot[2], slot[3]);
  const int4 cr = make_int4(comp_restart[0], comp_restart[1], comp_restart[2], comp_restart[3]);
  const int per_wg = 256 * STATS_DC_ITER;
  if (mcu_order) {
    const int rpw = (C.mcu_rows + 127) / 128;
    dim3 grid((C.mcu_rows + rpw - 1) / rpw, C.ncomp, n);
    hipLaunchKernelGGL(k_stats_dc_mcu, grid, dim3(256), 0, s, C, (const int16_t *)q, tabs, spi, sl, rpw);
  } else {
    dim3 grid((max_nblk(C) + per_wg - 1) / per_wg, C.ncomp, n);
    hipLaunchKernelGGL(k_stats_dc, grid, dim3(256), 0, s, C, (const int16_t *)q, tabs, spi, sl, cr);
  }
}

void mjh_launch_gen_tables(MjhHuffTable *tabs, int spi, const int *slots, int nslots, int n, hipStream_t s)
{
  int sl[8] = { 0, 0, 0, 0, 0, 0, 0, 0 };
  for (int i = 0; i < nslots && i < 8; i++) sl[i] = slots[i];
  hipLaunchKernelGGL(k_gen_tables, dim3(nslots, n), dim3(64), 0, s, tabs, spi, make_int4(sl[0], sl[1], sl[2], sl[3]), make_int4(sl[4], sl[5], sl[6], sl[7]));
}

void mjh_launch_gen_tables_list(MjhHuffTable *tabs, int spi, const int *d_slots, int nslots, int n, hipStream_t s)
{
  if (nslots > 0) hipLaunchKernelGGL(k_gen_tables_list, dim3(nslots, n), dim3(64), 0, s, tabs, spi, d_slots);
}

void mjh_launch_scan16(const void *len16, int n_per, unsigned *sums, int chunks, unsigned *totals, unsigned *off32, int npairs, hipStream_t s)
{
  hipLaunchKernelGGL((k_chunk_sums<uint16_t>), dim3(chunks, npairs), dim3(256), 0, s, (const uint16_t *)len16, n_per, sums, chunks);
  hipLaunchKernelGGL(k_scan_sums, dim3(npairs), dim3(256), 0, s, sums, chunks, totals, (const unsigned *)nullptr);
  hipLaunchKernelGGL((k_offsets<uint16_t>), dim3(chunks, npairs), dim3(256), 0, s, (const uint16_t *)len16, n_per, sums, chunks, off32);
}

bool mjh_trellis_dc_speculative_ok(const MjhConst &C, int window_ok)
{
  return window_ok && C.delta_dc_weight <= 0.0f && C.maxv >= 2;
}

void mjh_launch_trellis_dc_speculative(const MjhConst &C, const MjhQuant *Q, const void *uq, void *q, const MjhHuffTable *tabs, int spi, const int dc_slot[4], const float *lambda,
                                       void *back9, int *jfin, void *qspec, int n, hipStream_t s)
{
  int rows = 0;
  for (int c = 0; c < C.ncomp; c++) rows += C.c[c].hib;
  hipLaunchKernelGGL(k_trellis_dc3_fwd, dim3((rows * DC3_HYP + 3) / 4, n), dim3(64), 0, s, C, Q, (const int16_t *)uq, tabs, spi,
                     make_int4(dc_slot[0], dc_slot[1], dc_slot[2], dc_slot[3]), lambda, (uint8_t *)back9, jfin, (int16_t *)qspec, rows);
  hipLaunchKernelGGL(k_trellis_dc3_resolve, dim3(C.ncomp * C.mcu_rows, n), dim3(64), 0, s, C, (int16_t *)q, (const int *)jfin, (const int16_t *)qspec, rows);
}

void mjh_launch_trellis_dc(const MjhConst &C, const MjhQuant *Q, const void *uq, void *q, const MjhHuffTable *tabs, int spi, const int dc_slot[4], const float *lambda, void *back, int n, hipStream_t s,
                           int window_ok, int chain0, int chain1)
{
  const int nchains = C.ncomp * C.mcu_rows;
  if (chain1 < 0 || chain1 > nchains) chain1 = nchains;
  if (chain0 >= chain1) return;
  dim3 grid((chain1 - chain0 + 3) / 4, n);
  if (window_ok && C.delta_dc_weight <= 0.0f)
    hipLaunchKernelGGL(k_trellis_dc3, grid, dim3(64), 0, s, C, Q, (const int16_t *)uq, (int16_t *)q, tabs, spi, make_int4(dc_slot[0], dc_slot[1], dc_slot[2], dc_slot[3]), lambda, (uint8_t *)back, chain0, chain1);
  else hipLaunchKernelGGL(k_trellis_dc2, grid, dim3(64), 0, s, C, Q, (const int16_t *)uq, (int16_t *)q, tabs, spi, make_int4(dc_slot[0], dc_slot[1], dc_slot[2], dc_slot[3]), lambda, (uint8_t *)back, chain0, chain1);
}

void mjh_launch_encode(const MjhConst &C, const void *q, const unsigned long long *nzmask, const MjhHuffTable *tabs, int spi, const int dc_slot[4], const int ac_slot[4],
                       void *len16, void *off32, unsigned *sums, int chunks_per_image, unsigned *totals,
                       unsigned *stream, size_t stream_words_per_image, void *meta,
                       unsigned *seg_x, unsigned *seg_E, unsigned *seg_sums, unsigned *seg_totals, unsigned *mpos, int nseg,
                       int n, hipStream_t s)
{
  const int4 ds = make_int4(dc_slot[0], dc_slot[1], dc_slot[2], dc_slot[3]);
  const int4 as = make_int4(ac_slot[0], ac_slot[1], ac_slot[2], ac_slot[3]);
  dim3 grid((max_padblk(C) + 255) / 256, C.ncomp, n);
  if (nzmask) hipLaunchKernelGGL((k_enc_len<true>), grid, dim3(256), 0, s, C, (const int16_t *)q, nzmask, tabs, spi, ds, as, (uint16_t *)len16, (MjhImageMeta *)meta);
  else hipLaunchKernelGGL((k_enc_len<false>), grid, dim3(256), 0, s, C, (const int16_t *)q, nzmask, tabs, spi, ds, as, (uint16_t *)len16, (MjhImageMeta *)meta);
  hipLaunchKernelGGL((k_chunk_sums<uint16_t>), dim3(chunks_per_image, n), dim3(256), 0, s, (const uint16_t *)len16, C.total_mcu_blocks, sums, chunks_per_image);
  hipLaunchKernelGGL(k_scan_sums, dim3(n), dim3(256), 0, s, sums, chunks_per_image, totals, (const unsigned *)nullptr);
  hipLaunchKernelGGL((k_offsets<uint16_t>), dim3(chunks_per_image, n), dim3(256), 0, s, (const uint16_t *)len16, C.total_mcu_blocks, sums, chunks_per_image, (unsigned *)off32);
  const bool rst = C.restart_interval != 0 && nseg > 1;
  if (rst) {
    const int seg_chunks = (nseg + SCAN_CHUNK - 1) / SCAN_CHUNK;
    hipLaunchKernelGGL(k_seg_extra, dim3((nseg + 255) / 256, n), dim3(256), 0, s, C, (const unsigned *)off32, totals, seg_x, nseg);
    hipLaunchKernelGGL((k_chunk_sums<unsigned>), dim3(seg_chunks, n), dim3(256), 0, s, (const unsigned *)seg_x, nseg, seg_sums, seg_chunks);
    hipLaunchKernelGGL(k_scan_sums, dim3(n), dim3(256), 0, s, seg_sums, seg_chunks, seg_totals, (const unsigned *)nullptr);
    hipLaunchKernelGGL((k_offsets<unsigned>), dim3(seg_chunks, n), dim3(256), 0, s, (const unsigned *)seg_x, nseg, seg_sums, seg_chunks, seg_E);
  }
  hipLaunchKernelGGL(k_zero_stream, dim3(64, n), dim3(256), 0, s, stream, stream_words_per_image, (const unsigned *)totals,
                     rst ? (const unsigned *)seg_totals : (const unsigned *)nullptr);
  dim3 gridm((C.total_mcu_blocks + 255) / 256, n);
  if (nzmask) hipLaunchKernelGGL((k_enc_write_mcu<true>), gridm, dim3(256), 0, s, C, (const int16_t *)q, nzmask, tabs, spi, ds, as, (const unsigned *)off32, stream, stream_words_per_image,
                                 (const unsigned *)totals, (const unsigned *)seg_E, (const unsigned *)seg_totals, mpos, rst ? nseg : 1);
  else hipLaunchKernelGGL((k_enc_write_mcu<false>), gridm, dim3(256), 0, s, C, (const int16_t *)q, nzmask, tabs, spi, ds, as, (const unsigned *)off32, stream, stream_words_per_image,
                          (const unsigned *)totals, (const unsigned *)seg_E, (const unsigned *)seg_totals, mpos, rst ? nseg : 1);
  hipLaunchKernelGGL(k_finish_bits, dim3((n + 63) / 64), dim3(64), 0, s, totals, rst ? (const unsigned *)seg_totals : (const unsigned *)nullptr, stream,
                     stream_words_per_image, (MjhImageMeta *)meta, n);
}

__global__ void __launch_bounds__(64) k_spin(unsigned long long ticks, unsigned *sink)
{
  const unsigned long long t0 = wall_clock64();
  unsigned n = 0;
  while (wall_clock64() - t0 < ticks) n++;
  if (sink && threadIdx.x == 0 && n == 0xFFFFFFFFu) *sink = n;
}
void mjh_launch_spin(unsigned long long ticks, hipStream_t s) { hipLaunchKernelGGL(k_spin, dim3(1), dim3(64), 0, s, ticks, (unsigned *)nullptr); }

void mjh_launch_header(const void *prefix, int prefix_len, const void *sos, int sos_len, const MjhHuffTable *tabs, int spi,
                       const int dht_slots[8], const int dht_ids[8], int ndht, int multi_dht, void *out, size_t out_stride, void *meta, int n, hipStream_t s,
                       const unsigned *append_sizes)
{
  MjhDhtPlan plan;
  for (int i = 0; i < 8; i++) { plan.slots[i] = i < ndht ? dht_slots[i] : 0; plan.ids[i] = i < ndht ? dht_ids[i] : 0; }
  hipLaunchKernelGGL(k_header, dim3(n), dim3(64), 0, s, (const uint8_t *)prefix, prefix_len, (const uint8_t *)sos, sos_len, tabs, spi,
                     plan, ndht, multi_dht, (uint8_t *)out, out_stride, (MjhImageMeta *)meta, append_sizes);
}

void mjh_launch_finish_bits(unsigned *totals, unsigned *stream, size_t stream_words_per_image, void *meta, int n, hipStream_t s)
{
  hipLaunchKernelGGL(k_finish_bits, dim3((n + 63) / 64), dim3(64), 0, s, totals, (const unsigned *)nullptr, stream, stream_words_per_image, (MjhImageMeta *)meta, n);
}

void mjh_launch_stuff(const unsigned *stream, size_t stream_words_per_image, const unsigned *totals, unsigned *ffsums, int ff_chunks_per_image,
                      unsigned *ff_totals, void *out, size_t out_stride, void *meta, unsigned *sizes, const unsigned *mpos, int nseg, int n, hipStream_t s)
{
  int gx = 4096 / (n > 0 ? n : 1);
  if (gx < 128) gx = 128;
  if (gx > ff_chunks_per_image) gx = ff_chunks_per_image;
  hipLaunchKernelGGL(k_ff_chunk_sums, dim3(gx, n), dim3(256), 0, s, stream, stream_words_per_image, totals, ffsums, ff_chunks_per_image, mpos, nseg);
  hipLaunchKernelGGL(k_scan_sums, dim3(n), dim3(256), 0, s, ffsums, ff_chunks_per_image, ff_totals, totals);
  hipLaunchKernelGGL(k_stuff_write, dim3(gx, n), dim3(256), 0, s, stream, stream_words_per_image, totals, ffsums, ff_chunks_per_image,
                     ff_totals, (uint8_t *)out, out_stride, (MjhImageMeta *)meta, sizes, mpos, nseg);
}
```

### mozjpeg_amd/csrc/mjh_launch.h

```cpp
#ifndef MJH_LAUNCH_H
#define MJH_LAUNCH_H
#include <hip/hip_runtime.h>
#include "mjh_internal.h"

void mjh_launch_import_coefs(const MjhConst &C, const MjhCoefSrc &S, void *coef_q, void *meta, int n, hipStream_t s);
void mjh_launch_import_planes(const MjhConst &C, const MjhPlaneSrc &S, void *planes, int n, hipStream_t s);
void mjh_launch_color(const MjhConst &C, const void *pix, size_t row_pitch, size_t img_stride, void *planes, int n, hipStream_t s);
void mjh_launch_dct(const MjhConst &C, const MjhQuant *Q, const void *planes, void *uq, void *q, float *lambda,
                    MjhHuffTable *stat_tabs, int spi, const int stat_slot[4], uint8_t *nq8, int n, hipStream_t s, int fastdiv = 0, int ifast = 0);
void mjh_launch_stats_ac(const MjhConst &C, const void *q, const unsigned long long *nzmask, MjhHuffTable *tabs, int spi, const int slot[4], int count_dummies, int n, hipStream_t s);
void mjh_launch_stats_dc(const MjhConst &C, const void *q, MjhHuffTable *tabs, int spi, const int slot[4], int mcu_order, const int comp_restart[4], int n, hipStream_t s);
void mjh_launch_gen_tables(MjhHuffTable *tabs, int spi, const int *slots, int nslots, int n, hipStream_t s);
void mjh_launch_trellis_ac(const MjhConst &C, const MjhQuant *Q, const void *uq, void *q, MjhHuffTable *tabs, int spi, const int ac_slot[4], const float *lambda,
                           unsigned *worklist, unsigned *worklist2, void *dense, unsigned dense_cap, int variant,
                           int Ss, int Se, void *eob_cost, int *eob_has, unsigned long long *nzmask, int qstride, int n, hipStream_t s,
                           uint8_t *nq8 = nullptr, int v3_passes = 0, int fastdiv = 0, hipEvent_t after_first_tier = nullptr, hipEvent_t after_first_tier2 = nullptr,
                           int chunks = 1, hipStream_t side = nullptr, hipEvent_t *ev_chunk = nullptr, int count_mask = 0);
void mjh_launch_trellis_eob_chain(const MjhConst &C, void *q, const MjhHuffTable *tabs, int spi, const int ac_slot[4], const void *eob_cost, const int *eob_has,
                                  int Ss, int Se, int n, hipStream_t s);
void mjh_launch_qopt_accumulate(const MjhConst &C, const void *uq, const void *q, void *sums, int n, hipStream_t s);
void mjh_launch_qopt_update(void *sums, MjhQuant *Q, int n, hipStream_t s);
void mjh_launch_qopt_fix(const MjhQuant *Q, void *out, size_t out_stride, unsigned *sizes, int dqt_start, int sof_off, const int *tabs, int ntab,
                         int multi, int baseline_capable, int n, hipStream_t s);
void mjh_launch_trellis_dc(const MjhConst &C, const MjhQuant *Q, const void *uq, void *q, const MjhHuffTable *tabs, int spi, const int dc_slot[4], const float *lambda, void *back, int n, hipStream_t s,
                           int window_ok = 0, int chain0 = 0, int chain1 = -1);
void mjh_launch_encode(const MjhConst &C, const void *q, const unsigned long long *nzmask, const MjhHuffTable *tabs, int spi, const int dc_slot[4], const int ac_slot[4],
                       void *len16, void *off32, unsigned *sums, int chunks_per_image, unsigned *totals,
                       unsigned *stream, size_t stream_words_per_image, void *meta,
                       unsigned *seg_x, unsigned *seg_E, unsigned *seg_sums, unsigned *seg_totals, unsigned *mpos, int nseg,
                       int n, hipStream_t s);
void mjh_launch_header(const void *prefix, int prefix_len, const void *sos, int sos_len, const MjhHuffTable *tabs, int spi,
                       const int dht_slots[8], const int dht_ids[8], int ndht, int multi_dht, void *out, size_t out_stride, void *meta, int n, hipStream_t s, const unsigned *append_sizes = nullptr);
void mjh_launch_finish_bits(unsigned *totals, unsigned *stream, size_t stream_words_per_image, void *meta, int n, hipStream_t s);
void mjh_launch_stuff(const unsigned *stream, size_t stream_words_per_image, const unsigned *totals, unsigned *ffsums, int ff_chunks_per_image,
                      unsigned *ff_totals, void *out, size_t out_stride, void *meta, unsigned *sizes, const unsigned *mpos, int nseg, int n, hipStream_t s);
void mjh_launch_pack_results(const void *out, size_t out_stride, const unsigned *sizes, const void *meta, const void *prog_ctl, int n,
                             void *dst, size_t cap, void *table, hipStream_t s);
void mjh_launch_spin(unsigned long long ticks_100mhz, hipStream_t s);
void mjh_launch_gen_tables_list(MjhHuffTable *tabs, int spi, const int *d_slots, int nslots, int n, hipStream_t s);
void mjh_launch_prog_reset(void *ctl, int nscans, int n, hipStream_t s);
void mjh_launch_prog_stats(const MjhConst &C, const void *scans, const int *list, int nlist, void *ctl, const void *q,
                           MjhHuffTable *tabs, int spi, unsigned *mpos, int mpos_per_image, int n, hipStream_t s);
void mjh_launch_prog_stats_par(const MjhConst &C, const void *scans, const int *list, int nlist, void *ctl, const void *q,
                               MjhHuffTable *tabs, int spi, const MjhProgPE &pe, bool any_refine, const unsigned long long *nzmask, int n, hipStream_t s,
                               int nacf);
void mjh_launch_prog_encode(const MjhConst &C, const void *scans, const int *list, int nlist, const int *seq_list, int nseq,
                            const int *par_list, int npar, const MjhProgPE &pe, void *ctl, const void *q,
                            MjhHuffTable *tabs, int spi, unsigned *pool, size_t pool_words, const void *frame_hdr, int frame_hdr_len,
                            int multi_dht, void *outpool, size_t out_bytes, unsigned *mpos, int mpos_per_image, unsigned *ffsums, const unsigned long long *nzmask, int n, hipStream_t s,
                            hipStream_t side, hipEvent_t ev_fork, hipEvent_t ev_join, int nacf);
void mjh_launch_scan16(const void *len16, int n_per, unsigned *sums, int chunks, unsigned *totals, unsigned *off32, int npairs, hipStream_t s);
void mjh_launch_prog_select(void *ctl, int ncomp, int phase, int dc_scan_opt_mode, int n, hipStream_t s);
void mjh_launch_prog_concat(const void *ctl, const void *file_hdr, int file_hdr_len, const void *outpool, size_t out_bytes,
                            void *out, size_t out_stride, unsigned *sizes, int n, hipStream_t s);
bool mjh_trellis_dc_speculative_ok(const MjhConst &C, int window_ok);
void mjh_launch_trellis_dc_speculative(const MjhConst &C, const MjhQuant *Q, const void *uq, void *q, const MjhHuffTable *tabs, int spi, const int dc_slot[4], const float *lambda,
                                       void *back9, int *jfin, void *qspec, int n, hipStream_t s);
void mjh_launch_arith_scans(const MjhConst &C, const void *scans, const int *list, int nlist, void *ctl, const void *q,
                            const uint8_t *frame_hdr, int frame_hdr_len, const uint8_t *file_hdr, int file_hdr_len,
                            uint8_t *out, size_t out_stride, unsigned *sizes, int whole_blocks, int mode, int n, hipStream_t s);
void mjh_launch_arith_layout(void *ctl, const uint8_t *file_hdr, int file_hdr_len, uint8_t *out, size_t out_stride, unsigned *sizes, int n, hipStream_t s);
void mjh_launch_trellis_arith(const MjhConst &C, const MjhQuant *Q, int qstride, const void *uq, void *q, const float *lambda, const void *rate_tab, void *back,
                              int Ss, int Se, int quant_dc, float delta_dc_weight, int restart_blocks, int prog_file, int n, hipStream_t s);
#endif
```

Before: 145,200 Mpixels/s.

## Add one-pass Huffman encode with staged per-segment bit packing and placement

Replaces the two-pass Huffman encode (a length pass, a prefix scan, then a write pass) with a single pass. Each 256-block segment encodes its blocks into LDS staging and packs them into a per-segment word buffer. A separate kernel then shifts and places each segment into the final stream after a scan over segment totals. Blocks or segments that overflow the staging depth or window fall back to direct atomic writes or a separate recount-and-write kernel. It is enabled by default when there is no restart interval, and in exchange adds an extra packed buffer, more kernel launches and slow-path counters.

```diff
diff --git a/include/mozjpeg_hip.h b/include/mozjpeg_hip.h
--- a/include/mozjpeg_hip.h
+++ b/include/mozjpeg_hip.h
@@ -157,6 +157,8 @@
 int mjh_transcode_status(mjh_encoder *e, int i, const char **text);
 int mjh_transcode_stats(mjh_encoder *e, int *subseq, int *rounds, int *host_syncs, float ms[4]);
 
+int mjh_enc_onepass_stats(mjh_encoder *e, int *enabled, unsigned long long *long_blocks, unsigned long long *big_groups);
+
 int mjh_get_jpeg_size(mjh_encoder *e, int i, size_t *size);
 int mjh_get_jpeg(mjh_encoder *e, int i, void *dst, size_t cap, size_t *size);
 int mjh_get_output_device(mjh_encoder *e, void **d_base, size_t *stride, void **d_sizes);
diff --git a/mozjpeg_amd/__init__.py b/mozjpeg_amd/__init__.py
--- a/mozjpeg_amd/__init__.py
+++ b/mozjpeg_amd/__init__.py
@@ -137,6 +137,8 @@
         L.mjh_transcode_host.argtypes = [C.c_void_p, C.POINTER(C.c_char_p), C.POINTER(C.c_size_t), C.c_int]
         L.mjh_transcode_status.argtypes = [C.c_void_p, C.c_int, C.POINTER(C.c_char_p)]
         L.mjh_transcode_stats.argtypes = [C.c_void_p, C.POINTER(C.c_int), C.POINTER(C.c_int), C.POINTER(C.c_int), C.POINTER(C.c_float)]
+        if hasattr(L, "mjh_enc_onepass_stats"):
+            L.mjh_enc_onepass_stats.argtypes = [C.c_void_p, C.POINTER(C.c_int), C.POINTER(C.c_ulonglong), C.POINTER(C.c_ulonglong)]
         _lib = L
     return _lib
 
@@ -515,6 +517,11 @@
         _chk(lib().mjh_transcode_stats(self._h, C.byref(a), C.byref(b), C.byref(c), ms))
         return dict(subseq=a.value, rounds=b.value, host_syncs=c.value, ms=dict(zip(("sync", "prefix", "store", "dc"), [float(x) for x in ms])))
 
+    def enc_onepass_stats(self):
+        on, a, b = C.c_int(), C.c_ulonglong(), C.c_ulonglong()
+        _chk(lib().mjh_enc_onepass_stats(self._h, C.byref(on), C.byref(a), C.byref(b)))
+        return dict(enabled=bool(on.value), long_blocks=a.value, big_groups=b.value)
+
     def transcode_host(self, files, errors="raise"):
         n = len(files)
         try:
diff --git a/mozjpeg_amd/csrc/mjh_device.h b/mozjpeg_amd/csrc/mjh_device.h
--- a/mozjpeg_amd/csrc/mjh_device.h
+++ b/mozjpeg_amd/csrc/mjh_device.h
@@ -176,7 +176,7 @@
   __syncthreads();
 }
 
-template <bool LDSW>
+template <bool LDSW, bool SWAP = true>
 struct BitSink {
   unsigned *words;
   unsigned long long acc;
@@ -189,7 +189,7 @@
     nacc += n;
     if (nacc >= 32) {
       const unsigned w = (unsigned)(acc >> (nacc - 32));
-      atomicOr(&words[widx], __builtin_bswap32(w));
+      atomicOr(&words[widx], SWAP ? __builtin_bswap32(w) : w);
       widx++;
       nacc -= 32;
     }
@@ -201,16 +201,65 @@
     nacc += n;
     if (nacc >= 32) {
       const unsigned w = (unsigned)(acc >> (nacc - 32));
-      atomicOr(&words[widx], __builtin_bswap32(w));
+      atomicOr(&words[widx], SWAP ? __builtin_bswap32(w) : w);
       widx++;
       nacc -= 32;
     }
   }
   __device__ __forceinline__ void flush()
   {
-    if (nacc > 0) atomicOr(&words[widx], __builtin_bswap32((unsigned)(acc << (32 - nacc))));
+    if (nacc > 0) { const unsigned w = (unsigned)(acc << (32 - nacc)); atomicOr(&words[widx], SWAP ? __builtin_bswap32(w) : w); }
   }
   __device__ __forceinline__ unsigned bitpos() const { return widx * 32u + (unsigned)nacc; }
 };
 
+template <int DEPTH, int STRIDE>
+struct StageSink {
+  unsigned *col;
+  unsigned long long acc;
+  int nacc;
+  unsigned widx;
+  __device__ __forceinline__ void init(unsigned *c) { col = c; widx = 0; nacc = 0; acc = 0; }
+  __device__ __forceinline__ void put(unsigned code, int n)
+  {
+    acc = (acc << n) | (unsigned long long)(code & ((1u << n) - 1u));
+    nacc += n;
+    if (nacc >= 32) {
+      if (widx < (unsigned)DEPTH) col[widx * STRIDE] = (unsigned)(acc >> (nacc - 32));
+      widx++;
+      nacc -= 32;
+    }
+  }
+  __device__ __forceinline__ void put_sym(unsigned e, unsigned val, int nbits)
+  {
+    const int n = (int)(e >> 16) + nbits;
+    acc = (acc << n) | (unsigned long long)(((e & 0xFFFFu) << nbits) | (val & ((1u << nbits) - 1u)));
+    nacc += n;
+    if (nacc >= 32) {
+      if (widx < (unsigned)DEPTH) col[widx * STRIDE] = (unsigned)(acc >> (nacc - 32));
+      widx++;
+      nacc -= 32;
+    }
+  }
+  __device__ __forceinline__ void flush()
+  {
+    if (nacc > 0 && widx < (unsigned)DEPTH) col[widx * STRIDE] = (unsigned)(acc << (32 - nacc));
+  }
+  __device__ __forceinline__ unsigned bitpos() const { return widx * 32u + (unsigned)nacc; }
+};
+
+struct CountSink {
+  unsigned n;
+  __device__ __forceinline__ void init() { n = 0; }
+  __device__ __forceinline__ void put(unsigned, int k) { n += (unsigned)k; }
+  __device__ __forceinline__ void put_sym(unsigned e, unsigned, int nbits) { n += (e >> 16) + (unsigned)nbits; }
+  __device__ __forceinline__ void flush() {}
+  __device__ __forceinline__ unsigned bitpos() const { return n; }
+};
+
+__device__ __forceinline__ unsigned funnel_shift(unsigned hi, unsigned lo, unsigned s)
+{
+  return (unsigned)(((((unsigned long long)hi) << 32) | (unsigned long long)lo) >> s);
+}
+
 #endif
diff --git a/mozjpeg_amd/csrc/mjh_encoder.cpp b/mozjpeg_amd/csrc/mjh_encoder.cpp
--- a/mozjpeg_amd/csrc/mjh_encoder.cpp
+++ b/mozjpeg_amd/csrc/mjh_encoder.cpp
@@ -317,6 +317,10 @@
   unsigned *d_off32 = nullptr, *d_sums = nullptr, *d_totals = nullptr, *d_ffsums = nullptr, *d_fftotals = nullptr;
   unsigned *d_stream = nullptr;
   size_t stream_words = 0;
+  int enc_onepass = 1;
+  unsigned *d_pack = nullptr;
+  size_t pack_words = 0;
+  unsigned *d_enc_slow = nullptr;
   int chunks = 0, ff_chunks = 0;
   uint8_t *d_out = nullptr;
   size_t out_stride = 0;
@@ -756,7 +760,7 @@
   for (hipEvent_t ev : { e->ev_done, e->ev_tier1 }) if (ev) (void)hipEventDestroy(ev);
   if (e->ev_null_in) (void)hipEventDestroy(e->ev_null_in);
   void *ptrs[] = { e->d_pixb[0], e->d_pixb[1], e->d_plin, e->d_cfin, e->d_prog_mpos, e->d_prog_ffsums, e->d_prog_chunks, e->pe.len16, e->pe.run16, e->pe.tail16, e->pe.be16, e->pe.off32, e->pe.sums, e->pe.totals, e->pe.T32, e->pe.tsums, e->pe.ttotals, e->pe.ne_bits, e->pe.ne2_bits, e->pe.e_bits, e->pe.info, e->pe.chist, e->pe.rmask, e->d_planes, e->d_uq, e->d_q, e->d_q0, e->d_quant, e->d_quant_init, e->d_tabs, e->d_tabs_init, e->d_lambda, e->d_back, e->d_eob_cost, e->d_eob_has, e->d_qsums, e->d_nzmask, e->d_nq8, e->d_dense, e->d_worklist, e->d_worklist2, e->d_prog_scans, e->d_prog_ctl, e->d_lists, e->d_pool, e->d_outpool, e->d_frame_hdr, e->d_seg_x, e->d_seg_E, e->d_seg_sums, e->d_seg_totals, e->d_mpos,
-                   e->d_len16, e->d_off32, e->d_sums, e->d_totals, e->d_ffsums, e->d_fftotals, e->d_stream, e->d_out, e->d_sizes,
+                   e->d_len16, e->d_off32, e->d_pack, e->d_enc_slow, e->d_sums, e->d_totals, e->d_ffsums, e->d_fftotals, e->d_stream, e->d_out, e->d_sizes,
                    e->d_meta, e->d_prefix, e->d_sos, e->d_ll_hist, e->d_ll_len, e->d_ll_off, e->d_ll_segE, e->d_arith_rates, e->d_back9, e->d_jfin, e->d_qspec, e->g_in[0], e->g_in[1], e->g_in[2], e->g_in[3] };
   for (void *q : ptrs) if (q) (void)mjh_guard_free(q);
   for (void *q : e->g_in_old) (void)mjh_guard_free(q);
@@ -827,6 +831,7 @@
 }
 
 static thread_local bool g_create_twin = false;
+static thread_local int g_twin_onepass = 1;
 static thread_local hipStream_t g_twin_avoid[2] = { nullptr, nullptr };
 
 static hipError_t make_streams(mjh_encoder *e)
@@ -993,12 +998,20 @@
   HIPCHK_E(mjh_dmalloc((void **)&e->d_len16, B * (size_t)C.total_mcu_blocks * 2));
   HIPCHK_E(mjh_dmalloc((void **)&e->d_off32, B * (size_t)C.total_mcu_blocks * 4));
   e->chunks = (C.total_mcu_blocks + 2047) / 2048;
+  if (g_create_twin) e->enc_onepass = g_twin_onepass;
+  else if (const char *v = getenv("MJH_ENC_ONEPASS")) e->enc_onepass = atoi(v) != 0;
+  if (e->enc_onepass) {
+    e->pack_words = mjh_encode_pack_words(C);
+    HIPCHK_E(mjh_dmalloc((void **)&e->d_pack, B * e->pack_words * 4));
+    HIPCHK_E(mjh_dmalloc((void **)&e->d_enc_slow, 2 * sizeof(unsigned)));
+    HIPCHK_E(hipMemset(e->d_enc_slow, 0, 2 * sizeof(unsigned)));
+  }
   size_t words = (size_t)C.total_mcu_blocks * (C.precision == 12 ? 61 : 53) + 64;
   if (C.restart_interval) words += (size_t)(C.mcus_per_row * C.mcu_rows) / C.restart_interval + 1;
   if (words > (size_t)1 << 27) words = (size_t)1 << 27;
   e->stream_words = (words + 63) & ~(size_t)63;
   e->ff_chunks = (int)((e->stream_words + 2047) / 2048);
-  HIPCHK_E(mjh_dmalloc((void **)&e->d_sums, B * e->chunks * sizeof(unsigned)));
+  HIPCHK_E(mjh_dmalloc((void **)&e->d_sums, B * (size_t)std::max(e->chunks, mjh_encode_segments(C)) * sizeof(unsigned)));
   HIPCHK_E(mjh_dmalloc((void **)&e->d_ffsums, B * e->ff_chunks * sizeof(unsigned)));
   HIPCHK_E(mjh_dmalloc((void **)&e->d_totals, B * sizeof(unsigned)));
   HIPCHK_E(mjh_dmalloc((void **)&e->d_fftotals, B * sizeof(unsigned)));
@@ -1805,7 +1818,8 @@
                         p.compress_profile != MJH_PROFILE_FASTEST, e->d_out, e->out_stride, e->d_meta, n, s, si == 0 ? nullptr : e->d_sizes);
       pr.mark("huff_encode");
       mjh_launch_encode(V, e->d_q, nzm, e->d_tabs, spi, v_dc, v_ac, e->d_len16, e->d_off32, e->d_sums, e->chunks, e->d_totals,
-                        e->d_stream, e->stream_words, e->d_meta, e->d_seg_x, e->d_seg_E, e->d_seg_sums, e->d_seg_totals, e->d_mpos, q.nseg, n, s);
+                        e->d_stream, e->stream_words, e->d_meta, e->d_seg_x, e->d_seg_E, e->d_seg_sums, e->d_seg_totals, e->d_mpos, q.nseg, n, s,
+                        e->d_pack, e->pack_words, e->d_enc_slow);
       pr.mark("byte_stuff");
       mjh_launch_stuff(e->d_stream, e->stream_words, e->d_totals, e->d_ffsums, e->ff_chunks, e->d_fftotals, e->d_out, e->out_stride,
                        e->d_meta, e->d_sizes, e->d_mpos, q.nseg, n, s);
@@ -1831,7 +1845,8 @@
                       p.compress_profile != MJH_PROFILE_FASTEST, e->d_out, e->out_stride, e->d_meta, n, s);
     pr.mark("huff_encode");
     mjh_launch_encode(C, e->d_q, nzm, e->d_tabs, spi, fin_dc, fin_ac, e->d_len16, e->d_off32, e->d_sums, e->chunks, e->d_totals,
-                      e->d_stream, e->stream_words, e->d_meta, e->d_seg_x, e->d_seg_E, e->d_seg_sums, e->d_seg_totals, e->d_mpos, e->nseg, n, s);
+                      e->d_stream, e->stream_words, e->d_meta, e->d_seg_x, e->d_seg_E, e->d_seg_sums, e->d_seg_totals, e->d_mpos, e->nseg, n, s,
+                      e->d_pack, e->pack_words, e->d_enc_slow);
     if (if_mode == 2) { HIPCHK(hipEventRecord(e->ev_done, s)); e->ev_done_set = true; }
     pr.mark("byte_stuff");
     mjh_launch_stuff(e->d_stream, e->stream_words, e->d_totals, e->d_ffsums, e->ff_chunks, e->d_fftotals, e->d_out, e->out_stride,
@@ -1864,6 +1879,7 @@
 {
   mjh_encoder *t = nullptr;
   g_create_twin = true;
+  g_twin_onepass = e->enc_onepass;
   g_twin_avoid[0] = e->stream; g_twin_avoid[1] = e->side_stream;
   const int rc = mjh_encoder_create(&e->p_created, e->max_batch, e->device, &t);
   g_create_twin = false;
@@ -2709,6 +2725,24 @@
       for (int k = 0; k < 4; k++) HIPCHK(hipEventElapsedTime(&ms[k], e->tc_ev[k], e->tc_ev[k + 1]));
     }
   }
+  return MJH_OK;
+}
+
+extern "C" int mjh_enc_onepass_stats(mjh_encoder *e, int *enabled, unsigned long long *long_blocks, unsigned long long *big_groups)
+{
+  if (!e) return fail(MJH_EINVAL, "null encoder");
+  if (enabled) *enabled = e->enc_onepass;
+  unsigned long long a = 0, b = 0;
+  for (mjh_encoder *x : { e, e->twin }) {
+    if (!x || !x->d_enc_slow) continue;
+    unsigned h[2] = { 0, 0 };
+    HIPCHK(hipSetDevice(x->device));
+    HIPCHK(hipDeviceSynchronize());
+    HIPCHK(hipMemcpy(h, x->d_enc_slow, sizeof(h), hipMemcpyDeviceToHost));
+    a += h[0]; b += h[1];
+  }
+  if (long_blocks) *long_blocks = a;
+  if (big_groups) *big_groups = b;
   return MJH_OK;
 }
 
diff --git a/mozjpeg_amd/csrc/mjh_kernels.hip b/mozjpeg_amd/csrc/mjh_kernels.hip
--- a/mozjpeg_amd/csrc/mjh_kernels.hip
+++ b/mozjpeg_amd/csrc/mjh_kernels.hip
@@ -1733,7 +1733,8 @@
 
 template <bool COMPACT, class W>
 __device__ __forceinline__ void enc_write_block(const MjhConst &C, const MjhComp &cc, W &bw, const unsigned *s_ac, const unsigned *s_dc,
-                                                const int16_t *__restrict__ q, const unsigned long long *__restrict__ nzmask_img, int r, int c)
+                                                const int16_t *__restrict__ q, const unsigned long long *__restrict__ nzmask_img, int r, int c,
+                                                int *dc_nbits = nullptr)
 {
   const int dc = q[dc_source_block(cc, r, c)];
   int pr, pc, pred = 0;
@@ -1742,6 +1743,7 @@
     const int df = dc - pred;
     const int a = df < 0 ? -df : df;
     const int nb = bitlen((unsigned)a);
+    if (dc_nbits) *dc_nbits = nb;
     const unsigned e = s_dc[nb];
     bw.put(e & 0xFFFF, (int)(e >> 16));
     if (nb) bw.put((unsigned)(df < 0 ? df - 1 : df), nb);
@@ -1859,6 +1861,179 @@
     }
 }
 
+#define ENCP_DEPTH 8
+#define ENCP_WIN 2048
+
+__device__ __forceinline__ void enc_load_tables(unsigned (*s_ac)[256], unsigned (*s_dc)[32], const MjhConst &C, const MjhHuffTable *__restrict__ tabs_img,
+                                                const int4 &dc_slot_of_comp, const int4 &ac_slot_of_comp)
+{
+  const int tid = threadIdx.x;
+  for (int ci = 0; ci < C.ncomp; ci++) {
+    const int dslot = ci == 0 ? dc_slot_of_comp.x : ci == 1 ? dc_slot_of_comp.y : ci == 2 ? dc_slot_of_comp.z : dc_slot_of_comp.w;
+    const int aslot = ci == 0 ? ac_slot_of_comp.x : ci == 1 ? ac_slot_of_comp.y : ci == 2 ? ac_slot_of_comp.z : ac_slot_of_comp.w;
+    const MjhHuffTable *TD = tabs_img + dslot;
+    const MjhHuffTable *TA = tabs_img + aslot;
+    s_ac[ci][tid] = ((unsigned)TA->ehufsi[tid] << 16) | TA->ehufco[tid];
+    if (tid < 32) s_dc[ci][tid] = tid < 16 ? ((unsigned)TD->ehufsi[tid] << 16) | TD->ehufco[tid] : 0u;
+  }
+}
+
+__device__ __forceinline__ int enc_scan_position(const MjhConst &C, int p, int &r, int &c)
+{
+  const int mcu = p / C.blocks_per_mcu, bi = p - mcu * C.blocks_per_mcu;
+  int comp = 0;
+  for (int ci = 1; ci < C.ncomp; ci++) if (bi >= C.c[ci].mcu_blk0) comp = ci;
+  const int h = C.c[comp].h, v = C.c[comp].v;
+  const int local = bi - C.c[comp].mcu_blk0, yi = local / h, xi = local - yi * h;
+  const int mrow = mcu / C.mcus_per_row, mcol = mcu - mrow * C.mcus_per_row;
+  r = mrow * v + yi;
+  c = mcol * h + xi;
+  return comp;
+}
+
+template <bool COMPACT>
+__global__ void __launch_bounds__(256)
+k_enc_write_pack(MjhConst C, const int16_t *__restrict__ coef_q, const unsigned long long *__restrict__ nzmask, const MjhHuffTable *__restrict__ tabs,
+                 int slots_per_image, int4 dc_slot_of_comp, int4 ac_slot_of_comp,
+                 unsigned *__restrict__ pack, size_t pack_words_per_image, unsigned *__restrict__ sums, int segs_per_image,
+                 MjhImageMeta *__restrict__ meta, unsigned *__restrict__ slow)
+{
+  __shared__ unsigned s_ac[MJH_MAXC][256];
+  __shared__ unsigned s_dc[MJH_MAXC][32];
+  __shared__ unsigned s_stage[ENCP_DEPTH * 256];
+  __shared__ uint4 s_win4[ENCP_WIN / 4];
+  __shared__ unsigned sh[8];
+  unsigned *s_win = reinterpret_cast<unsigned *>(s_win4);
+  const int img = blockIdx.y, tid = threadIdx.x;
+  const int N = C.total_mcu_blocks, p = blockIdx.x * 256 + tid;
+  enc_load_tables(s_ac, s_dc, C, tabs + (size_t)img * slots_per_image, dc_slot_of_comp, ac_slot_of_comp);
+  for (int i = tid; i < ENCP_WIN / 4; i += 256) s_win4[i] = make_uint4(0u, 0u, 0u, 0u);
+  __syncthreads();
+  int r = 0, c = 0;
+  const int comp = enc_scan_position(C, p < N ? p : 0, r, c);
+  const MjhComp cc = C.c[comp];
+  const int16_t *q = coef_q + (size_t)img * C.coefs_per_image + cc.coef_off;
+  const unsigned long long *nzi = COMPACT ? nzmask + (size_t)img * C.total_real_blocks : nullptr;
+  unsigned bits = 0;
+  if (p < N) {
+    MJH_DIVERGENT_SCOPE;
+    StageSink<ENCP_DEPTH, 256> bw;
+    bw.init(s_stage + tid);
+    int nb = 0;
+    enc_write_block<COMPACT>(C, cc, bw, s_ac[comp], s_dc[comp], q, nzi, r, c, &nb);
+    bw.flush();
+    bits = bw.bitpos();
+    if (nb > (C.precision == 12 ? 15 : 11)) meta[img].bad_coef = 1u;
+  }
+  unsigned tot;
+  const unsigned ex = block_excl_scan_256_1b(bits, sh, 0, &tot);
+  if (tid == 0) sums[(size_t)img * segs_per_image + blockIdx.x] = tot;
+  const unsigned nw = (tot + 31u) >> 5;
+  if (nw > (unsigned)ENCP_WIN) {
+    if (tid == 0) atomicAdd(&slow[1], 1u);
+    return;
+  }
+  if (bits > ENCP_DEPTH * 32u) {
+    MJH_DIVERGENT_SCOPE;
+    atomicAdd(&slow[0], 1u);
+    BitSink<true, false> bw;
+    bw.init(s_win, ex);
+    enc_write_block<COMPACT>(C, cc, bw, s_ac[comp], s_dc[comp], q, nzi, r, c);
+    bw.flush();
+  } else {
+    const unsigned s = ex & 31u, w0 = ex >> 5, nsw = (bits + 31u) >> 5, ndw = (s + bits + 31u) >> 5;
+    unsigned prev = 0u;
+    for (unsigned k = 0; k < ndw; k++) {
+      const unsigned cur = k < nsw ? s_stage[k * 256 + tid] : 0u;
+      const unsigned v = funnel_shift(prev, cur, s);
+      if (v) atomicOr(&s_win[w0 + k], v);
+      prev = cur;
+    }
+  }
+  __syncthreads();
+  unsigned *g = pack + (size_t)img * pack_words_per_image + (size_t)blockIdx.x * ENCP_WIN;
+  for (unsigned i = tid; i < nw; i += 256) g[i] = s_win[i];
+}
+
+__global__ void __launch_bounds__(256)
+k_enc_write_place(const unsigned *__restrict__ pack, size_t pack_words_per_image, const unsigned *__restrict__ sums, int segs_per_image,
+                  const unsigned *__restrict__ totals, unsigned *__restrict__ stream, size_t stream_words_per_image)
+{
+  const int img = blockIdx.y, lane = threadIdx.x & 63;
+  const int seg = blockIdx.x * 4 + (threadIdx.x >> 6);
+  if (seg >= segs_per_image) return;
+  const unsigned total = totals[img];
+  if (total == 0xFFFFFFFFu) return;
+  const unsigned *sm = sums + (size_t)img * segs_per_image;
+  const unsigned base = sm[seg], len = (seg + 1 < segs_per_image ? sm[seg + 1] : total) - base;
+  const unsigned nsw = (len + 31u) >> 5;
+  if (nsw > (unsigned)ENCP_WIN) return;
+  const unsigned s = base & 31u, ndw = (s + len + 31u) >> 5;
+  const unsigned *src = pack + (size_t)img * pack_words_per_image + (size_t)seg * ENCP_WIN;
+  unsigned *g = stream + (size_t)img * stream_words_per_image + (base >> 5);
+  for (unsigned k = lane; k < ndw; k += 64) {
+    const unsigned hi = k > 0u ? src[k - 1] : 0u, lo = k < nsw ? src[k] : 0u;
+    const unsigned v = __builtin_bswap32(funnel_shift(hi, lo, s));
+    if (k == 0u || k == ndw - 1u) { if (v) atomicOr(&g[k], v); }
+    else g[k] = v;
+  }
+}
+
+template <bool COMPACT>
+__global__ void __launch_bounds__(256)
+k_enc_write_big(MjhConst C, const int16_t *__restrict__ coef_q, const unsigned long long *__restrict__ nzmask, const MjhHuffTable *__restrict__ tabs,
+                int slots_per_image, int4 dc_slot_of_comp, int4 ac_slot_of_comp, const unsigned *__restrict__ sums, int segs_per_image,
+                const unsigned *__restrict__ totals, unsigned *__restrict__ stream, size_t stream_words_per_image)
+{
+  __shared__ unsigned s_ac[MJH_MAXC][256];
+  __shared__ unsigned s_dc[MJH_MAXC][32];
+  __shared__ unsigned sh[4];
+  __shared__ unsigned s_base[256];
+  const int img = blockIdx.y, tid = threadIdx.x, N = C.total_mcu_blocks;
+  const unsigned total = totals[img];
+  if (total == 0xFFFFFFFFu) return;
+  const unsigned *sm = sums + (size_t)img * segs_per_image;
+  unsigned *g = stream + (size_t)img * stream_words_per_image;
+  const int seg0 = blockIdx.x * 256;
+  unsigned mine = 0xFFFFFFFFu;
+  if (seg0 + tid < segs_per_image) {
+    const int sg = seg0 + tid;
+    const unsigned base = sm[sg], len = (sg + 1 < segs_per_image ? sm[sg + 1] : total) - base;
+    if (((len + 31u) >> 5) > (unsigned)ENCP_WIN) mine = base;
+  }
+  s_base[tid] = mine;
+  if (!__syncthreads_or(mine != 0xFFFFFFFFu)) return;
+  enc_load_tables(s_ac, s_dc, C, tabs + (size_t)img * slots_per_image, dc_slot_of_comp, ac_slot_of_comp);
+  __syncthreads();
+  for (int i = 0; i < 256 && seg0 + i < segs_per_image; i++) {
+    const unsigned base = s_base[i];
+    if (base == 0xFFFFFFFFu) continue;
+    const int seg = seg0 + i;
+    const int p = seg * 256 + tid;
+    int r = 0, c = 0;
+    const int comp = enc_scan_position(C, p < N ? p : 0, r, c);
+    const MjhComp cc = C.c[comp];
+    const int16_t *q = coef_q + (size_t)img * C.coefs_per_image + cc.coef_off;
+    const unsigned long long *nzi = COMPACT ? nzmask + (size_t)img * C.total_real_blocks : nullptr;
+    unsigned bits = 0;
+    if (p < N) {
+      MJH_DIVERGENT_SCOPE;
+      CountSink cs;
+      cs.init();
+      enc_write_block<COMPACT>(C, cc, cs, s_ac[comp], s_dc[comp], q, nzi, r, c);
+      bits = cs.bitpos();
+    }
+    const unsigned ex = block_excl_scan_256(bits, sh, nullptr);
+    if (p < N) {
+      MJH_DIVERGENT_SCOPE;
+      BitSink<false> bw;
+      bw.init(g, base + ex);
+      enc_write_block<COMPACT>(C, cc, bw, s_ac[comp], s_dc[comp], q, nzi, r, c);
+      bw.flush();
+    }
+  }
+}
+
 __global__ void __launch_bounds__(256)
 k_zero_stream(unsigned *__restrict__ stream, size_t stream_words_per_image, const unsigned *__restrict__ totals,
               const unsigned *__restrict__ seg_totals)
@@ -2123,6 +2298,9 @@
 #undef LC
 }
 
+int mjh_encode_segments(const MjhConst &C) { return (C.total_mcu_blocks + 255) / 256; }
+size_t mjh_encode_pack_words(const MjhConst &C) { return (size_t)mjh_encode_segments(C) * ENCP_WIN; }
+
 static int max_nblk(const MjhConst &C) { int m = 0; for (int i = 0; i < C.ncomp; i++) m = C.c[i].nblk > m ? C.c[i].nblk : m; return m; }
 static int max_padblk(const MjhConst &C) { int m = 0; for (int i = 0; i < C.ncomp; i++) { int v = C.c[i].wpad * C.c[i].hpad; m = v > m ? v : m; } return m; }
 
@@ -2213,10 +2391,29 @@
                        void *len16, void *off32, unsigned *sums, int chunks_per_image, unsigned *totals,
                        unsigned *stream, size_t stream_words_per_image, void *meta,
                        unsigned *seg_x, unsigned *seg_E, unsigned *seg_sums, unsigned *seg_totals, unsigned *mpos, int nseg,
-                       int n, hipStream_t s)
+                       int n, hipStream_t s, unsigned *pack, size_t pack_words_per_image, unsigned *slow)
 {
   const int4 ds = make_int4(dc_slot[0], dc_slot[1], dc_slot[2], dc_slot[3]);
   const int4 as = make_int4(ac_slot[0], ac_slot[1], ac_slot[2], ac_slot[3]);
+  if (pack && C.restart_interval == 0) {
+    const int segs = mjh_encode_segments(C);
+    dim3 gridp(segs, n);
+    if (nzmask) hipLaunchKernelGGL((k_enc_write_pack<true>), gridp, dim3(256), 0, s, C, (const int16_t *)q, nzmask, tabs, spi, ds, as, pack, pack_words_per_image, sums, segs,
+                                   (MjhImageMeta *)meta, slow);
+    else hipLaunchKernelGGL((k_enc_write_pack<false>), gridp, dim3(256), 0, s, C, (const int16_t *)q, nzmask, tabs, spi, ds, as, pack, pack_words_per_image, sums, segs,
+                            (MjhImageMeta *)meta, slow);
+    hipLaunchKernelGGL(k_scan_sums, dim3(n), dim3(256), 0, s, sums, segs, totals, (const unsigned *)nullptr);
+    hipLaunchKernelGGL(k_zero_stream, dim3(64, n), dim3(256), 0, s, stream, stream_words_per_image, (const unsigned *)totals, (const unsigned *)nullptr);
+    hipLaunchKernelGGL(k_enc_write_place, dim3((segs + 3) / 4, n), dim3(256), 0, s, (const unsigned *)pack, pack_words_per_image, (const unsigned *)sums, segs,
+                       (const unsigned *)totals, stream, stream_words_per_image);
+    dim3 gridb((segs + 255) / 256, n);
+    if (nzmask) hipLaunchKernelGGL((k_enc_write_big<true>), gridb, dim3(256), 0, s, C, (const int16_t *)q, nzmask, tabs, spi, ds, as, (const unsigned *)sums, segs,
+                                   (const unsigned *)totals, stream, stream_words_per_image);
+    else hipLaunchKernelGGL((k_enc_write_big<false>), gridb, dim3(256), 0, s, C, (const int16_t *)q, nzmask, tabs, spi, ds, as, (const unsigned *)sums, segs,
+                            (const unsigned *)totals, stream, stream_words_per_image);
+    hipLaunchKernelGGL(k_finish_bits, dim3((n + 63) / 64), dim3(64), 0, s, totals, (const unsigned *)nullptr, stream, stream_words_per_image, (MjhImageMeta *)meta, n);
+    return;
+  }
   dim3 grid((max_padblk(C) + 255) / 256, C.ncomp, n);
   if (nzmask) hipLaunchKernelGGL((k_enc_len<true>), grid, dim3(256), 0, s, C, (const int16_t *)q, nzmask, tabs, spi, ds, as, (uint16_t *)len16, (MjhImageMeta *)meta);
   else hipLaunchKernelGGL((k_enc_len<false>), grid, dim3(256), 0, s, C, (const int16_t *)q, nzmask, tabs, spi, ds, as, (uint16_t *)len16, (MjhImageMeta *)meta);
diff --git a/mozjpeg_amd/csrc/mjh_launch.h b/mozjpeg_amd/csrc/mjh_launch.h
--- a/mozjpeg_amd/csrc/mjh_launch.h
+++ b/mozjpeg_amd/csrc/mjh_launch.h
@@ -28,7 +28,9 @@
                        void *len16, void *off32, unsigned *sums, int chunks_per_image, unsigned *totals,
                        unsigned *stream, size_t stream_words_per_image, void *meta,
                        unsigned *seg_x, unsigned *seg_E, unsigned *seg_sums, unsigned *seg_totals, unsigned *mpos, int nseg,
-                       int n, hipStream_t s);
+                       int n, hipStream_t s, unsigned *pack = nullptr, size_t pack_words_per_image = 0, unsigned *slow = nullptr);
+int mjh_encode_segments(const MjhConst &C);
+size_t mjh_encode_pack_words(const MjhConst &C);
 void mjh_launch_header(const void *prefix, int prefix_len, const void *sos, int sos_len, const MjhHuffTable *tabs, int spi,
                        const int dht_slots[8], const int dht_ids[8], int ndht, int multi_dht, void *out, size_t out_stride, void *meta, int n, hipStream_t s, const unsigned *append_sizes = nullptr);
 void mjh_launch_finish_bits(unsigned *totals, unsigned *stream, size_t stream_words_per_image, void *meta, int n, hipStream_t s);
```

After: 149,900 Mpixels/s (median of 6 runs). +3.2%, better.
